# Yukayo/MobGT

Hardware: AMD Instinct MI355X
Metric: check-ins/sec (train step) (higher is better)
Workload: dtype bf16

## Files before the change

__graft_entry__.py:

```python
import os
import subprocess
import sys

ROOT = os.path.dirname(os.path.abspath(__file__))
if ROOT not in sys.path:
    sys.path.insert(0, ROOT)


def build() -> None:
    from mobgt_amd import _native
    for library in _native.LIBRARIES:
        library.build()
        library.lib()
    from mobgt_amd import _pairbins
    _pairbins.LIBRARY.build()
    _pairbins.LIBRARY.lib()
    from mobgt_amd import _universe
    _universe.LIBRARY.build()
    _universe.LIBRARY.lib()
    subprocess.check_call(["make", "-s", "-C", os.path.join(ROOT, "oracle")])
    import mobgt_amd


def smoke() -> None:
    import numpy as np
    import torch
    from mobgt_amd import ops, synth
    from mobgt_amd.model_fqandtoyo import EncoderLayer
    from oracle import algos_oracle as ao
    from oracle import model_oracle as mo
    assert torch.cuda.is_available(), "smoke() needs cuda:0"
    dev = "cuda:0"
    G, H, T, C = 3, 8, 37, 192
    torch.manual_seed(0)
    layer = EncoderLayer(C, 256, 0.1, 0.1, H).eval()
    sd = {"L." + k: v.detach().clone().requires_grad_(True) for k, v in layer.state_dict().items()}
    rng = np.random.RandomState(0)
    x = torch.from_numpy(rng.standard_normal((G, T, C)).astype(np.float32))
    gy = torch.from_numpy(rng.standard_normal((G, T, C)).astype(np.float32))
    bias = torch.from_numpy((rng.standard_normal((G, H, T, T)) * 0.5).astype(np.float32))
    bias[1, :, :, 30:] = float("-inf")
    xr, br = x.clone().requires_grad_(True), bias.clone().requires_grad_(True)
    ref = mo.encoder_layer_fq(sd, "L", xr, br, H)
    ref.backward(gy)
    layer = layer.to(dev)
    xd, bd = x.to(dev).requires_grad_(True), bias.to(dev).requires_grad_(True)
    out = layer(xd, bd)
    out.backward(gy.to(dev))
    torch.cuda.synchronize()

    def close(name, got, want, tol):
        got, want = got.detach().float().cpu().numpy(), want.detach().numpy()
        scale = float(np.sqrt((want ** 2).mean()))
        err = float(np.abs(got - want).max())
        assert err <= tol * scale, f"{name}: max |err| {err:.3e} vs rms {scale:.3e}"
    close("y", out, ref, 1e-3)
    close("dx", xd.grad, xr.grad, 1e-3)
    close("dbias", bd.grad, br.grad, 1e-3)
    for k, p in layer.named_parameters():
        if k.endswith("linear_k.bias"):
            continue
        if sd["L." + k].grad is not None:
            close("d" + k, p.grad, sd["L." + k].grad, 2e-3)
    layer.act_dtype = torch.bfloat16
    for prm in layer.parameters():
        prm.grad = None
    xb, bb = x.to(dev).requires_grad_(True), bias.to(dev).requires_grad_(True)
    out16 = layer(xb, bb)
    out16.backward(gy.to(dev))
    torch.cuda.synchronize()
    close("y (bf16)", out16, ref, 8e-2)
    close("dx (bf16)", xb.grad, xr.grad, 1e-1)
    close("dbias (bf16)", bb.grad, br.grad, 2e-1)
    trajs = synth.make_batch_of_trajectories(seed=4, G=4, P=50, n_user=8, n_nodes=[17, 3, 9, 30])
    n = np.array([len(t["node_name"]) for t in trajs], dtype=np.int32)
    counts = np.zeros((4, 30, 30), dtype=np.int32)
    for g, t in enumerate(trajs):
        counts[g, :n[g], :n[g]] = t["edge_type"]
    sp = ops.spd_batched(torch.from_numpy(counts).to(dev), torch.from_numpy(n).to(dev), 20)
    for g in range(4):
        k = int(n[g])
        M, path = ao.floyd_warshall(counts[g, :k, :k] != 0)
        assert np.array_equal(sp["spd"][g, :k, :k].cpu().numpy().astype(np.int64), M)
        assert np.array_equal(sp["path"][g, :k, :k].cpu().numpy().astype(np.int64), path)
    print("smoke ok: fused fq EncoderLayer fwd+bwd (f32 and bf16 configurations) and batched SPD match the oracle")


if __name__ == "__main__":
    build()
    if len(sys.argv) > 1 and sys.argv[1] == "smoke":
        smoke()
```

mobgt_amd/csrc/tokbwd.hip:

```cpp
#include "common.h"
#include "mobgt_hip.h"

namespace {

typedef __attribute__((ext_vector_type(4))) float f32x4;

constexpr int TNW = 12, TNT = TNW * 64, TBM = 16;

struct TokBwdParams {
    const float* dout;
    const float* real;
    const float* y4;
    const float* y2; int64_t ld2;
    const float *w4, *w2;
    float *d_nf, *d_add;
    float* dx4; int64_t ldx4;
    float* d_pt;
    float* d_token;
    int G, N;
    float slope4, slope2;
    uint32_t thr_pos, thr_in;
    float keep_pos, keep_in;
    uint64_t seed;
    const uint64_t* seed_dev;
    uint32_t salt_nf, salt_tok, salt_in;
    int n_node_blocks;
};

__device__ __forceinline__ float leaky_grad(float y, float slope) { return y > 0.f ? 1.f : slope; }

#ifdef TB_STAMP
__device__ int* g_tb_dbg = nullptr;
#define TSTAMP_DECL int st_[8] = {}
#define TSTAMP(i) st_[i] = (int)wall_clock64()
#define TSTAMP_DUMP() do { if (g_tb_dbg && threadIdx.x == 0) for (int q_ = 0; q_ < 8; ++q_) g_tb_dbg[blockIdx.x * 8 + q_] = st_[q_]; } while (0)
#else
#define TSTAMP_DECL
#define TSTAMP(i)
#define TSTAMP_DUMP()
#endif

template <int N> constexpr int gemm_ks() { return TNW / ((N + 63) / 64); }
template <int K, int N, int LDA, int LDO>
__device__ __forceinline__ void gemm_kn(const float* __restrict__ A, const float* __restrict__ W, float* __restrict__ out) {
    constexpr int NB = (N + 63) / 64, KS = TNW / NB, NT16 = K / 16, TMAX = (NT16 + KS - 1) / KS;
    static_assert(K % 16 == 0 && N % 32 == 0 && KS >= 1, "shape");
    const int lane = threadIdx.x & 63, wave = threadIdx.x >> 6;
    const int j = lane & 15, q = lane >> 4;
    if (wave >= NB * KS) return;
    const int blk = wave / KS, ks = wave % KS;
    const int t_lo = ks * NT16 / KS, t_hi = (ks + 1) * NT16 / KS;
    const int n0 = 64 * blk;
    const bool col_ok = n0 + 4 * j < N;
    const int cl = col_ok ? n0 + 4 * j : 0;
    f32x4 acc[4];
#pragma unroll
    for (int n = 0; n < 4; ++n) acc[n] = f32x4{0.f, 0.f, 0.f, 0.f};
    f32x4 bw[TMAX][4];
#pragma unroll
    for (int tt = 0; tt < TMAX; ++tt) {
        const int t = min(t_lo + tt, t_hi - 1);
#pragma unroll
        for (int i = 0; i < 4; ++i) bw[tt][i] = *reinterpret_cast<const f32x4*>(W + (int64_t)(16 * t + 4 * q + i) * N + cl);
    }
#pragma unroll
    for (int tt = 0; tt < TMAX; ++tt) {
        if (t_lo + tt < t_hi) {
            const f32x4 a = *reinterpret_cast<const f32x4*>(A + j * LDA + 16 * (t_lo + tt) + 4 * q);
#pragma unroll
            for (int i = 0; i < 4; ++i)
#pragma unroll
                for (int n = 0; n < 4; ++n) acc[n] = __builtin_amdgcn_mfma_f32_16x16x4f32(a[i], bw[tt][i][n], acc[n], 0, 0, 0);
        }
    }
    if (col_ok) {
#pragma unroll
        for (int n = 0; n < 4; ++n)
#pragma unroll
            for (int v = 0; v < 4; ++v) out[(ks * TBM + 4 * q + v) * LDO + n0 + 4 * j + n] = acc[n][v];
    }
}

template <int C, int W2>
__global__ __launch_bounds__(TNT) void token_bwd_chain_kernel(const TokBwdParams p) {
    constexpr int LDA = C + 4, LD2 = W2 + 4;
    __shared__ __attribute__((aligned(16))) float a4[TBM * LDA];
    constexpr int KS4 = gemm_ks<C>(), KS2 = gemm_ks<W2>();
    __shared__ __attribute__((aligned(16))) float t4[(KS4 > KS2 ? KS4 : KS2) * TBM * LDA];
    const int lane = threadIdx.x & 63, wave = threadIdx.x >> 6;
    const int T = p.N + 1;
    const uint64_t seed = (p.thr_pos || p.thr_in) ? p.seed + (p.seed_dev ? *p.seed_dev : 0ull) : 0ull;
    if ((int)blockIdx.x >= p.n_node_blocks) {
        const int g = ((int)blockIdx.x - p.n_node_blocks) * TNW + wave;
        if (g >= p.G) return;
        const int64_t row = (int64_t)g * T;
        const uint32_t h1 = p.thr_pos ? dropout_row_hash(seed, (uint32_t)g ^ p.salt_tok) : 0u;
        const uint32_t h2 = p.thr_in ? dropout_row_hash(seed, (uint32_t)row ^ p.salt_in) : 0u;
        for (int c = lane; c < C; c += 64) {
            float scale = 1.f;
            if (p.thr_pos) scale = dropout_bits16(seed, h1, (uint32_t)c) >= p.thr_pos ? p.keep_pos : 0.f;
            if (p.thr_in) scale *= dropout_bits16(seed, h2, (uint32_t)c) >= p.thr_in ? p.keep_in : 0.f;
            const float d = p.dout[row * C + c] * scale;
            if (d != 0.f) atomicAdd(&p.d_token[c], d);
        }
        return;
    }
    const int64_t R = (int64_t)p.G * p.N;
    const int64_t j0 = (int64_t)blockIdx.x * TBM;
    TSTAMP_DECL;
    TSTAMP(0);
    constexpr int EPT = TBM * C / TNT;
    static_assert(TBM * C % TNT == 0, "flat split");
    float dv[EPT], yv[EPT], rl[EPT];
#pragma unroll
    for (int k = 0; k < EPT; ++k) {
        const int e = threadIdx.x + k * TNT, r = e / C, c = e % C;
        const int64_t jc = min(j0 + r, R - 1);
        const int g = (int)(jc / p.N), n = (int)(jc - (int64_t)g * p.N);
        dv[k] = p.dout[((int64_t)g * T + n + 1) * C + c];
        yv[k] = p.y4[jc * C + c];
        rl[k] = p.real[jc];
    }
#pragma unroll
    for (int k = 0; k < EPT; ++k) {
        const int e = threadIdx.x + k * TNT, r = e / C, c = e % C;
        const int64_t jn = j0 + r;
        const bool on = jn < R;
        const int64_t jc = on ? jn : R - 1;
        const int g = (int)(jc / p.N), n = (int)(jc - (int64_t)g * p.N);
        const int64_t row = (int64_t)g * T + n + 1;
        float scale = 1.f;
        if (p.thr_pos) scale = dropout_bits16(seed, dropout_row_hash(seed, (uint32_t)jc ^ p.salt_nf), (uint32_t)c) >= p.thr_pos ? p.keep_pos : 0.f;
        if (p.thr_in) scale *= dropout_bits16(seed, dropout_row_hash(seed, (uint32_t)row ^ p.salt_in), (uint32_t)c) >= p.thr_in ? p.keep_in : 0.f;
        const float d = on ? dv[k] * scale : 0.f;
        const float dnf = d * rl[k];
        a4[r * LDA + c] = dnf * leaky_grad(yv[k], p.slope4);
        if (on) {
            p.d_add[jn * C + c] = d;
            p.d_nf[jn * C + c] = dnf;
        }
    }
    __syncthreads();
    TSTAMP(1);
    gemm_kn<C, C, LDA, LDA>(a4, p.w4, t4);
    __syncthreads();
    TSTAMP(2);
    for (int e = threadIdx.x; e < TBM * C; e += TNT) {
        const int r = e / C, c = e % C;
        const int64_t jn = j0 + r;
        float v = 0.f;
#pragma unroll
        for (int ks = 0; ks < KS4; ++ks) v += t4[(ks * TBM + r) * LDA + c];
        if (jn < R) p.dx4[jn * p.ldx4 + c] = v;
        if (c < W2) a4[r * LD2 + c] = jn < R ? v * leaky_grad(p.y2[jn * p.ld2 + c], p.slope2) : 0.f;
    }
    __syncthreads();
    TSTAMP(3);
    gemm_kn<W2, W2, LD2, LD2>(a4, p.w2, t4);
    __syncthreads();
    TSTAMP(4);
    for (int e = threadIdx.x; e < TBM * W2; e += TNT) {
        const int r = e / W2, c = e % W2;
        const int64_t jn = j0 + r;
        float v = 0.f;
#pragma unroll
        for (int ks = 0; ks < KS2; ++ks) v += t4[(ks * TBM + r) * LD2 + c];
        if (jn < R) p.d_pt[jn * W2 + c] = v;
    }
    TSTAMP(5);
    TSTAMP_DUMP();
}

}

#ifdef TB_STAMP
extern "C" int mobgt_tokbwd_debug_buffer(int* buf) { return (int)hipMemcpyToSymbol(HIP_SYMBOL(g_tb_dbg), &buf, sizeof(buf)); }
#endif

extern "C" int mobgt_token_bwd_chain(const float* dout, const float* real, const float* y4, const float* y2, int64_t ld_y2,
                                     const float* w4, const float* w2, float* d_nf, float* d_add, float* dx4, int64_t ld_dx4,
                                     float* d_pt, float* d_token, int G, int N, int C, int W2, float slope4, float slope2,
                                     float p_pos, float p_in, uint64_t seed, const uint64_t* seed_dev, uint32_t salt_nf,
                                     uint32_t salt_tok, uint32_t salt_in, void* stream) {
    if (G <= 0 || N <= 0) return MOBGT_EBADDIM;
    if (!(C == 192 && W2 == 160)) return MOBGT_EBADDIM;
    if (((uintptr_t)w4 | (uintptr_t)w2) & 15) return MOBGT_EALIGN;
    TokBwdParams p = {};
    p.dout = dout; p.real = real; p.y4 = y4; p.y2 = y2; p.ld2 = ld_y2; p.w4 = w4; p.w2 = w2; p.d_nf = d_nf; p.d_add = d_add;
    p.dx4 = dx4; p.ldx4 = ld_dx4; p.d_pt = d_pt; p.d_token = d_token; p.G = G; p.N = N; p.slope4 = slope4; p.slope2 = slope2;
    p.thr_pos = p_pos > 0.f ? dropout_threshold(p_pos) : 0u;
    p.thr_in = p_in > 0.f ? dropout_threshold(p_in) : 0u;
    p.keep_pos = p.thr_pos ? 1.f / (1.f - (float)p.thr_pos / 65536.f) : 1.f;
    p.keep_in = p.thr_in ? 1.f / (1.f - (float)p.thr_in / 65536.f) : 1.f;
    p.seed = seed; p.seed_dev = seed_dev; p.salt_nf = salt_nf; p.salt_tok = salt_tok; p.salt_in = salt_in;
    p.n_node_blocks = (int)(((int64_t)G * N + TBM - 1) / TBM);
    const dim3 grid(p.n_node_blocks + (G + TNW - 1) / TNW), block(TNT);
    hipLaunchKernelGGL((token_bwd_chain_kernel<192, 160>), grid, block, 0, (hipStream_t)stream, p);
    return (int)hipGetLastError();
}
```

mobgt_amd/forms.py:

```python
import contextlib
import os
from collections import namedtuple

Form = namedtuple("Form", "name env default doc")

_ROWS = (
    Form("safe_forms", "MOBGT_SAFE_FORMS", False, "no launch waits for peer workgroups: one workgroup per row block, the head as "
         "three launches, the GCN layer by layer (what TrainStep.guarded_step switches to before it re-runs a faulted step)"),
    Form("chain", "MOBGT_NO_CHAIN", True, "out-proj -> LN -> FFN -> LN -> the next layer's QKV in one launch (off: separate launches)"),
    Form("chain_big", "MOBGT_NO_CHAIN_BIG", True, "past 4 096 rows: the 64-row forward chain (off: the library's GEMMs)"),
    Form("chain_bwd", None, True, "the same chain backwards, d(out) -> d(attention out)"),
    Form("ln_gemm", None, True, "dropout+residual+LN as the prologue of the GEMM that consumes it (off: the two-launch form)"),
    Form("ln_gemm_bwd", "MOBGT_LN_GEMM_BWD", False, "the LayerNorm-prologue GEMMs in the backward as well"),
    Form("own_gemm", None, True, "the layer's GEMMs on csrc/gemm.hip (off: through torch)"),
    Form("tail", None, True, "a layer's input-gradient GEMM rides in its grouped weight-gradient launch"),
    Form("defer_tail", "MOBGT_NO_DEFER_TAIL", True, "a layer leaves dx and its weight gradients to the chain_bwd launch of the layer "
         "below (off: it finishes its own backward)"),
    Form("wgrad_big", None, True, "past 4 096 rows: the layer's weight gradients as one launch"),
    Form("skinny_all", "MOBGT_SKINNY_ALL", False, "all three classifier products on csrc/skinny.hip (off: dW / db only)"),
    Form("token_fwd_chain", "MOBGT_NO_TOKEN_FWD_CHAIN", True, "the encoder input's forward as one launch (off: four)"),
    Form("token_bwd_chain", "MOBGT_NO_TOKEN_BWD_CHAIN", True, "the encoder input's backward as one launch, csrc/tokbwd.hip (off: three)"),
    Form("pack_passenger", "MOBGT_NO_PACK_PASSENGER", True, "the layers' weight pack, in the next front launch"),
    Form("front_passengers", "MOBGT_NO_FRONT_PASSENGERS", True, "hop table forward and node-feature indices, in the category GCN's forward"),
    Form("bias_bwd_passenger", "MOBGT_NO_BIAS_BWD_PASSENGER", True, "short batches: the bias tables' backward, in the category GCN's backward"),
    Form("bias_bwd_beside", None, True, "long batches: the bias tables' backward on a side stream (off: where autograd reaches it)"),
    Form("l0_ride", "MOBGT_NO_L0_RIDE", True, "the distance GCN's first product, in the bias assembly's launch"),
    Form("psum_defer", "MOBGT_NO_PSUM_DEFER", True, "split-K partial sums, in the step's one reduction launch into the gradient sinks"),
    Form("small_gcn", "MOBGT_NO_SMALL_GCN", True, "the three-layer category GCN as one launch each way (off: layer by layer)"),
    Form("conv_act", "MOBGT_NO_CONV_ACT", True, "bias + LeakyReLU + dropout in the small GEMM's epilogue (off: launch per product)"),
    Form("dist_gcn_fused", "MOBGT_NO_DIST_GCN_FUSED", True, "the distance GCN on the masked-GEMM launches"),
    Form("sp_gather", None, True, "sparse adjacency, transposed product as a gather (off: the atomic scatter)"),
    Form("stock_front", "MOBGT_NO_STOCK_FRONT", True, "hop table, weight pack and encoder input as one front launch"),
    Form("stock_tail", "MOBGT_NO_STOCK_TAIL", True, "the encoder input's and the wide hop table's backward share one grid at the flush"),
    Form("stock_ln_qkv", "MOBGT_NO_STOCK_LN_QKV", True, "the first layer's norm inside its QKV GEMM"),
    Form("attn_one_pass", "MOBGT_ATTN_TWO_PASS", True, "T > 64, bf16: one-pass backward (off: the two deterministic passes)"),
    Form("ddp_overlap", "MOBGT_DDP_OVERLAP", False, "the backward split into graphs, finished gradient slices all-reduced beside the next"),
    Form("ddp_host_exchange", "MOBGT_DDP_HOST_EXCHANGE", False, "all-reduce issued by the host between backward and optimizer graph"),
    Form("force_comm", "MOBGT_FORCE_COMM", False, "a process group of one rank takes the data-parallel path (tests)"),
)
_BY_NAME = {row.name: row for row in _ROWS}
_OVERRIDES = {}


def _env_set(var):
    v = os.environ.get(var, "")
    if v in ("", "0"):
        return False
    if v == "1":
        return True
    raise ValueError(f"{var}={v!r}: expected unset, '', '0' or '1'")


def on(name):
    row = _BY_NAME[name]
    if name in _OVERRIDES:
        return _OVERRIDES[name]
    if row.env is not None and _env_set(row.env):
        return not row.default
    return row.default


def set(name, value):
    _BY_NAME[name]
    if value is None:
        _OVERRIDES.pop(name, None)
    else:
        _OVERRIDES[name] = bool(value)


@contextlib.contextmanager
def using(**names):
    saved = dict(_OVERRIDES)
    try:
        for name, value in names.items():
            set(name, value)
        yield
    finally:
        _OVERRIDES.clear()
        _OVERRIDES.update(saved)


def table():
    return _ROWS
```

mobgt_amd/ops.py:

```python
import contextlib
import ctypes
import math

import torch

from . import _lib, forms
from ._lib import F32, BF16, I64, I32, I16, U8, check
from .step_state import STEP

_DT = {torch.float32: F32, torch.bfloat16: BF16}
_IT = {torch.int64: I64, torch.int32: I32, torch.int16: I16, torch.uint8: U8}


def _stream():
    return ctypes.c_void_p(torch.cuda.current_stream().cuda_stream)


def _p(t):
    return ctypes.c_void_p(t.data_ptr()) if t is not None else ctypes.c_void_p(0)


def _require_cuda(*ts):
    for t in ts:
        if t is not None and not t.is_cuda:
            raise RuntimeError("mobgt_amd ops run on the GPU only (there is no CPU fallback); got a CPU tensor")




def _ws_word(ws, off):
    return ws.view(torch.int32)[off // 4:off // 4 + 1]


def _scrub_exchange_area(ws, fault_off):
    ws[fault_off + 4:].zero_()
    torch.cuda.synchronize()


def peer_wait_faults(reset=True):
    from . import fused_layer
    lib = _lib.lib()
    dev = torch.cuda.current_device()
    torch.cuda.synchronize(dev)
    out = {}
    for key, ws in fused_layer._CHAIN_WS.items():
        if key[0] != dev:
            continue
        off = int(lib.mobgt_chain_ws_fault_offset())
        w = _ws_word(ws, off)
        n = int(w.item())
        if n:
            out["chain"] = out.get("chain", 0) + n
            if reset:
                w.zero_()
                _scrub_exchange_area(ws, off)
    ws = _HEAD_WS.get(dev)
    if ws is not None:
        off = int(lib.mobgt_head_chain_ws_fault_offset())
        w = _ws_word(ws, off)
        n = int(w.item())
        if n:
            out["head"] = n
            if reset:
                w.zero_()
                _scrub_exchange_area(ws, off)
    c = ctypes.c_uint32(0)
    _lib.call("mobgt_small_gcn_faults", 1 if reset else 0, ctypes.byref(c))
    if c.value:
        out["small_gcn"] = int(c.value)
    return out


def set_peer_wait_limit(rounds=0, gcn_ticks=0):
    from . import fused_layer
    lib = _lib.lib()
    dev = torch.cuda.current_device()
    rounds = int(rounds) & 0xFFFFFFFF
    rounds = rounds - (1 << 32) if rounds >= (1 << 31) else rounds
    for key, ws in fused_layer._CHAIN_WS.items():
        if key[0] == dev:
            _ws_word(ws, int(lib.mobgt_chain_ws_limit_offset())).fill_(int(rounds))
    ws = _HEAD_WS.get(dev)
    if ws is not None:
        _ws_word(ws, int(lib.mobgt_head_chain_ws_limit_offset())).fill_(int(rounds))
    _lib.call("mobgt_small_gcn_set_wait_limit", int(gcn_ticks))
    torch.cuda.synchronize()


class ZeroArena:

    def __init__(self, device, n=1 << 20):
        self.buf = torch.zeros(n, dtype=torch.float32, device=device)
        self.off = 0

    def reset(self):
        self.buf.zero_()
        self.off = 0

    def take(self, n):
        n4 = (n + 3) // 4 * 4
        if self.off + n4 > self.buf.numel():
            return None
        t = self.buf[self.off:self.off + n]
        self.off += n4
        return t


def set_zero_arena(arena):
    STEP.zero_arena = arena


def zeros_f32(shape, device):
    n = 1
    for d in (shape if isinstance(shape, (tuple, list, torch.Size)) else (shape,)):
        n *= int(d)
    a = STEP.zero_arena
    if a is not None and a.buf.device == torch.device(device):
        t = a.take(n)
        if t is not None:
            return t.view(shape)
    return torch.zeros(shape, dtype=torch.float32, device=device)


def set_grad_sinks(params, views):
    import weakref
    STEP.grad_sinks = {p.data_ptr(): (weakref.ref(p), v) for p, v in zip(params, views)} if params is not None else {}


def sink_census_begin():
    STEP.sink_census.update(on=True, cur={}, max={})


def sink_census_pass():
    c = STEP.sink_census
    for k, n in c["cur"].items():
        if n > c["max"].get(k, 0):
            c["max"][k] = n
    c["cur"] = {}


def sink_census_end():
    sink_census_pass()
    c = STEP.sink_census
    out, c["on"], c["max"] = c["max"], False, {}
    return out


def grad_sink(param):
    c = STEP.sink_census
    if c["on"]:
        c["cur"][id(param)] = c["cur"].get(id(param), 0) + 1
    e = STEP.grad_sinks.get(param.data_ptr())
    if e is not None and e[0]() is param and e[1].shape == param.shape:
        return e[1]
    return None


def round_up(x, m):
    return (x + m - 1) // m * m


class PackedBias:

    def __init__(self, G, H, T, dtype, device):
        self.G, self.H, self.T = G, H, T
        self.ld = round_up(T, 64)
        self.dtype = dtype
        self.bias = torch.empty(G, H, T, self.ld, dtype=dtype, device=device)
        self.bias_t = torch.empty(G, H, T, self.ld, dtype=dtype, device=device)
        self.dbias = None
        self.n_use = 0
        self.n_bwd = 0
        self.needs_grad = False
        self.token = None
        self.spent = False

    def dense(self):
        return self.bias[..., : self.T].float()

    @property
    def sliced(self):
        return self.dtype == torch.bfloat16

    def grad_buffer(self):
        if self.dbias is None:
            shape = (self.G, self.H, self.T, self.ld)
            if self.sliced:
                self.dbias = torch.empty((max(self.n_use, 1),) + shape, dtype=torch.bfloat16, device=self.bias.device)
            else:
                self.dbias = torch.zeros(shape, dtype=torch.float32, device=self.bias.device)
        return self.dbias

    def next_grad_slice(self):
        buf = self.grad_buffer()
        i = self.n_bwd
        self.n_bwd += 1
        if not self.sliced:
            return buf, 1 if i > 0 else 0
        if i >= buf.shape[0]:
            raise RuntimeError("PackedBias: more attention backward passes than forward uses of this bias")
        return buf[i], 0

    def grad_total(self):
        if self.dbias is None:
            return None
        if self.sliced:
            return self.dbias[: max(self.n_bwd, 1), ..., : self.T].float().sum(0)
        return self.dbias[..., : self.T]


class _PackFn(torch.autograd.Function):
    @staticmethod
    def forward(ctx, src, pack):
        G, H, T = pack.G, pack.H, pack.T
        s = src.expand(G, H, T, T)
        st = s.stride()
        _lib.call("mobgt_bias_pack", _p(s), _DT[s.dtype], st[0], st[1], st[2], st[3], _p(pack.bias), _p(pack.bias_t),
                  _DT[pack.dtype], G, H, T, pack.ld, _stream())
        ctx.pack = pack
        ctx.src_shape = src.shape
        ctx.src_dtype = src.dtype
        ctx.set_materialize_grads(False)
        return zeros_f32((1,), src.device)

    @staticmethod
    def backward(ctx, _g):
        pack = ctx.pack
        pack.spent = True
        if pack.dbias is None:
            return torch.zeros(ctx.src_shape, dtype=ctx.src_dtype, device=pack.bias.device), None
        g = pack.grad_total()
        if tuple(ctx.src_shape) != tuple(g.shape):
            g = g.sum_to_size(ctx.src_shape)
        return g.to(ctx.src_dtype), None


def pack_bias(attn_bias, G, H, T, dtype=None):
    _require_cuda(attn_bias)
    if attn_bias.dtype not in _DT:
        attn_bias = attn_bias.float()
    if attn_bias.dim() == 3:
        attn_bias = attn_bias.unsqueeze(1)
    pack = PackedBias(G, H, T, dtype or attn_bias.dtype, attn_bias.device)
    pack.needs_grad = attn_bias.requires_grad and torch.is_grad_enabled()
    pack.token = _PackFn.apply(attn_bias, pack)
    return pack




def front_deferral(on):
    STEP.front_on = bool(on) and forms.on("front_passengers")


def take_front_jobs():
    hop, ni = STEP.front_hop, STEP.front_ni
    STEP.front_hop = STEP.front_ni = None
    return hop, ni


def flush_front():
    hop, ni = take_front_jobs()
    if hop is not None:
        _lib.call("mobgt_hop_table_fwd", *hop[0], _stream())
    if ni is not None:
        _lib.call("mobgt_node_index", *ni[0], _stream())


def _bias_bwd_alloc(shapes, dev, sinks=(None, None, None, None)):
    return tuple(None if sh is None else (k[:] if (k is not None and tuple(k.shape) == tuple(sh)) else zeros_f32(sh, dev))
                 for sh, k in zip(shapes, sinks))


def take_bias_bwd_job():
    job, STEP.bias_bwd_job = STEP.bias_bwd_job, None
    if job is None or not forms.on("bias_bwd_passenger"):
        return None
    pack = job["pack"]()
    if pack is None or pack.dbias is None or not pack.sliced or pack.n_use < 1 or pack.n_bwd < pack.n_use:
        return None
    G, N, H, D_in, D, F, n_rel, n_poi, n_edge, ld, idx_dt, edge_dt = job["args"]
    if not (idx_dt == I16 and edge_dt == U8 and H == 8 and D > 0 and D <= 20 and F == 1 and G * (N + 1) * (N + 1) < (1 << 20)
            and job["idx"][3] is not None):
        return None
    return job


def bias_bwd_job_args(job):
    pack = job["pack"]()
    outs = _bias_bwd_alloc(job["shapes"], pack.bias.device, job.get("sinks", (None,) * 4))
    attn_bias, rel_pos, poi_pos, edge_input = job["idx"]
    n_sl = max(pack.n_bwd, 1) if pack.sliced else 1
    stride = pack.dbias.stride(0) if pack.sliced else 0
    args = [_p(pack.dbias), _DT[pack.dbias.dtype], n_sl, stride, _p(attn_bias), _p(rel_pos), _p(poi_pos), _p(edge_input),
            _p(outs[0]), _p(outs[1]), _p(outs[2]), _p(outs[3]), *job["args"]]
    return outs, args


class _BuildBiasFn(torch.autograd.Function):
    @staticmethod
    def forward(ctx, rel_table, poi_table, hop_table, vdist, pack, attn_bias, rel_pos, poi_pos, edge_input, D, sinks=(None,) * 4):
        G, N = rel_pos.shape[:2]
        H = rel_table.shape[1]
        has_edge = edge_input is not None and D > 0
        D_in = edge_input.shape[3] if has_edge else 0
        F = edge_input.shape[4] if has_edge else 1
        idx_dt = _IT[rel_pos.dtype]
        edge_dt = _IT[edge_input.dtype] if has_edge else U8
        n_poi = poi_table.shape[0] if poi_table is not None else 0
        n_edge = hop_table.shape[1] if has_edge else 0
        args = (G, N, H, D_in, D if has_edge else 0, F, rel_table.shape[0], n_poi, n_edge, pack.ld, idx_dt, edge_dt)
        _lib.call("mobgt_build_bias", _p(attn_bias), _p(rel_pos), _p(poi_pos), _p(edge_input if has_edge else None), _p(rel_table),
                  _p(poi_table), _p(hop_table if has_edge else None), _p(vdist), _p(pack.bias), _p(pack.bias_t),
                  *args, _DT[pack.dtype], _stream())
        ctx.pack, ctx.args = pack, args
        ctx.set_materialize_grads(False)
        ctx.idx = (attn_bias, rel_pos, poi_pos, edge_input if has_edge else None)
        ctx.shapes = (rel_table.shape, None if poi_table is None else poi_table.shape,
                      hop_table.shape if has_edge else None, vdist.shape)
        import weakref
        ctx.job = dict(pack=weakref.ref(pack), args=args, idx=ctx.idx, shapes=ctx.shapes, done=None, sinks=sinks)
        STEP.bias_bwd_job = ctx.job if pack.needs_grad else None
        return zeros_f32((1,), rel_table.device)

    @staticmethod
    def backward(ctx, _g):
        pack = ctx.pack
        dev = pack.bias.device
        if ctx.job["done"] is not None:
            d_rel, d_poi, d_hop, d_vd = ctx.job["done"]
            ev = ctx.job.pop("done_event", None)
            if ev is not None:
                torch.cuda.current_stream(pack.bias.device).wait_event(ev)
            ctx.job["done"] = None
            return d_rel, d_poi, d_hop, d_vd, None, None, None, None, None, None, None
        if STEP.bias_bwd_job is ctx.job:
            STEP.bias_bwd_job = None
        d_rel, d_poi, d_hop, d_vd = _bias_bwd_alloc(ctx.shapes, dev, ctx.job.get("sinks", (None,) * 4))
        if pack.dbias is not None:
            attn_bias, rel_pos, poi_pos, edge_input = ctx.idx
            a = ctx.args
            n_sl = max(pack.n_bwd, 1) if pack.sliced else 1
            stride = pack.dbias.stride(0) if pack.sliced else 0
            _lib.call("mobgt_build_bias_bwd", _p(pack.dbias), _DT[pack.dbias.dtype], n_sl, stride,
                      _p(attn_bias), _p(rel_pos), _p(poi_pos), _p(edge_input),
                      _p(d_rel), _p(d_poi), _p(d_hop), _p(d_vd), *a, _stream())
        return d_rel, d_poi, d_hop, d_vd, None, None, None, None, None, None, None


def build_bias(attn_bias, rel_pos, poi_pos, edge_input, rel_table, poi_table, hop_table, vdist, D, dtype=torch.float32):
    _require_cuda(attn_bias, rel_pos, rel_table)
    G, N = rel_pos.shape[:2]
    H = rel_table.shape[1]
    pack = PackedBias(G, H, N + 1, dtype, rel_table.device)
    pack.needs_grad = torch.is_grad_enabled() and any(
        t is not None and t.requires_grad for t in (rel_table, poi_table, hop_table, vdist))
    f = lambda t: None if t is None else t.contiguous()
    k_vd = grad_sink(vdist)
    sinks = (grad_sink(rel_table), grad_sink(poi_table) if poi_table is not None else None, None,
             k_vd.view(-1) if (k_vd is not None and k_vd.is_contiguous()) else None)
    pack.token = _BuildBiasFn.apply(f(rel_table.float()), f(None if poi_table is None else poi_table.float()),
                                    f(None if hop_table is None else hop_table.float()), f(vdist.float().reshape(-1)),
                                    pack, f(attn_bias.float()), f(rel_pos), f(poi_pos), f(edge_input), int(D), sinks)
    return pack


_ATTN_ONE_PASS = type("_AttnOnePassView", (), {"__getitem__": lambda self, i: forms.on("attn_one_pass")})()


def _check_rows(*ts):
    for t in ts:
        if t.stride(-1) != 1 or t.stride(-2) % 8 != 0 or t.data_ptr() % 16 != 0:
            raise RuntimeError("mobgt attention: q/k/v rows must be unit-stride, 16-byte aligned, row stride % 8 == 0")


def _lse_alloc(G, H, T, C, dtype, device):
    return torch.empty(lse_numel(G, H, T, C, dtype), dtype=torch.float32, device=device)


def lse_numel(G, H, T, C, dtype):
    n = G * H * T
    extra = (G * T * C + 1) // 2 if dtype == torch.bfloat16 else 0
    return (n + 3) // 4 * 4 + extra


def lse_rows(lse, G, H, T):
    return lse[: G * H * T].view(G, H, T)


def _out_lo_ptr(lse, G, H, T, dtype):
    if dtype != torch.bfloat16:
        return None
    return lse.data_ptr() + 4 * ((G * H * T + 3) // 4 * 4)


def _attn_fwd(q, k, v, pack, scale, p_drop, seed, seed_dev):
    G, T, C = q.shape
    H = pack.H
    out = torch.empty(G, T, C, dtype=q.dtype, device=q.device)
    lse = _lse_alloc(G, H, T, C, q.dtype, q.device)
    _check_rows(q, k, v)
    if pack.needs_grad:
        pack.n_use += 1
    _lib.call("mobgt_attn_bias_fwd", _p(q), _p(k), _p(v), _p(pack.bias), _p(out), _out_lo_ptr(lse, G, H, T, q.dtype), _p(lse), G, H, T, C // H,
              q.stride(1), k.stride(1), v.stride(1), C, pack.ld, scale, p_drop, seed,
              _p(seed_dev), _DT[q.dtype], _DT[pack.dtype], _stream())
    return out, lse


_DQ_ACC = {}
_DQ_ACC_RETIRED = []


def _attn_bwd(q, k, v, out, lse, dout, dq, dk, dv, pack, scale, p_drop, seed, seed_dev):
    G, T, C = q.shape
    H = pack.H
    need = lse_numel(G, H, T, C, q.dtype) if q.dtype == torch.bfloat16 else G * H * T
    if lse.dtype != torch.float32 or lse.numel() < need:
        raise ValueError(f"attention backward: `lse` must be the float32 buffer of {need} elements the "
                         f"forward returned (log-sum-exp rows + the bf16 residual of `out`), got {lse.dtype} x {lse.numel()}")
    dbias = None
    acc = 0
    if pack.needs_grad:
        dbias, acc = pack.next_grad_slice()
    delta = torch.empty(G, H, T, dtype=torch.float32, device=q.device)
    args = (_p(q), _p(k), _p(v), _p(pack.bias), _p(pack.bias_t), _p(out), _out_lo_ptr(lse, G, H, T, q.dtype), _p(lse), _p(dout),
            _p(dq), _p(dk), _p(dv), _p(dbias), _p(delta), G, H, T, C // H,
            q.stride(1), k.stride(1), v.stride(1), C, dq.stride(1), dk.stride(1),
            dv.stride(1), pack.ld, scale, p_drop, seed, _p(seed_dev), acc,
            _DT[dbias.dtype] if dbias is not None else F32, _DT[q.dtype], _DT[pack.dtype])
    if (T > 64 and q.dtype == torch.bfloat16 and pack.dtype == torch.bfloat16 and dbias is not None
            and dbias.dtype == torch.bfloat16 and _ATTN_ONE_PASS[0]):
        key = (str(q.device), int(torch.cuda.current_stream(q.device).cuda_stream), G * T * C)
        ent = _DQ_ACC.get(key)
        if ent is None or ent["busy"]:
            if ent is not None:
                _DQ_ACC_RETIRED.append(ent["buf"])
            ent = _DQ_ACC[key] = dict(buf=torch.zeros(G * T * C, dtype=torch.float32, device=q.device), busy=False)
        ent["busy"] = True
        _lib.call("mobgt_attn_bias_bwd_fused_z", *args, _p(ent["buf"]), _stream())
        ent["busy"] = False
        _bias_bwd_beside(pack)
        return
    _lib.call("mobgt_attn_bias_bwd", *args, _stream())
    _bias_bwd_beside(pack)


_SIDE_STREAMS = {}


def _bias_bwd_beside(pack):
    job = STEP.bias_bwd_job
    if (job is None or not forms.on("bias_bwd_beside") or job["pack"]() is not pack or not pack.sliced or pack.dbias is None
            or pack.n_use < 1 or pack.n_bwd < pack.n_use or job["done"] is not None):
        return
    G, N = job["args"][0], job["args"][1]
    if G * (N + 1) * (N + 1) < (1 << 20) or job["idx"][3] is None:
        return
    dev = pack.bias.device
    main = torch.cuda.current_stream(dev)
    side = _SIDE_STREAMS.get(dev)
    if side is None:
        side = _SIDE_STREAMS[dev] = torch.cuda.Stream(device=dev)
    STEP.bias_bwd_job = None
    outs, args = bias_bwd_job_args(job)
    fork = torch.cuda.Event()
    fork.record(main)
    side.wait_event(fork)
    cus = torch.cuda.get_device_properties(dev).multi_processor_count
    lib = _lib.lib()
    lib.mobgt_build_bias_bwd_set_workgroups(max(1, cus * 3 // 4))
    try:
        _lib.call("mobgt_build_bias_bwd", *args, ctypes.c_void_p(side.cuda_stream))
    finally:
        lib.mobgt_build_bias_bwd_set_workgroups(0)
    done = torch.cuda.Event()
    done.record(side)
    job["done"], job["done_event"] = outs, done


class _AttnFn(torch.autograd.Function):

    @staticmethod
    def forward(ctx, q, k, v, token, pack, scale, p_drop, seed, seed_dev):
        out, lse = _attn_fwd(q, k, v, pack, scale, p_drop, seed, seed_dev)
        ctx.save_for_backward(q, k, v, out, lse)
        ctx.misc = (pack, scale, p_drop, seed, seed_dev)
        return out

    @staticmethod
    def backward(ctx, dout):
        q, k, v, out, lse = ctx.saved_tensors
        pack, scale, p_drop, seed, seed_dev = ctx.misc
        dout = dout.contiguous()
        dq, dk, dv = torch.empty_like(out), torch.empty_like(out), torch.empty_like(out)
        _attn_bwd(q, k, v, out, lse, dout, dq, dk, dv, pack, scale, p_drop, seed, seed_dev)
        return dq, dk, dv, None, None, None, None, None, None


class _AttnQKVFn(torch.autograd.Function):

    @staticmethod
    def forward(ctx, qkv, token, pack, scale, p_drop, seed, seed_dev):
        C = qkv.shape[2] // 3
        q, k, v = qkv[..., :C], qkv[..., C:2 * C], qkv[..., 2 * C:]
        out, lse = _attn_fwd(q, k, v, pack, scale, p_drop, seed, seed_dev)
        ctx.save_for_backward(qkv, out, lse)
        ctx.misc = (pack, scale, p_drop, seed, seed_dev)
        return out

    @staticmethod
    def backward(ctx, dout):
        qkv, out, lse = ctx.saved_tensors
        pack, scale, p_drop, seed, seed_dev = ctx.misc
        C = qkv.shape[2] // 3
        q, k, v = qkv[..., :C], qkv[..., C:2 * C], qkv[..., 2 * C:]
        dqkv = torch.empty_like(qkv)
        _attn_bwd(q, k, v, out, lse, dout.contiguous(), dqkv[..., :C], dqkv[..., C:2 * C], dqkv[..., 2 * C:], pack,
                  scale, p_drop, seed, seed_dev)
        return dqkv, None, None, None, None, None, None


def attention(q, k, v, pack, scale, p_drop=0.0, seed=0, seed_dev=None):
    _require_cuda(q, k, v)
    return _AttnFn.apply(q, k, v, pack.token, pack, float(scale), float(p_drop), int(seed), seed_dev)


def attention_qkv(qkv, pack, scale, p_drop=0.0, seed=0, seed_dev=None):
    _require_cuda(qkv)
    if qkv.shape[2] % 24 != 0:
        raise RuntimeError("fused qkv width must be 3*C with C % 8 == 0")
    return _AttnQKVFn.apply(qkv.contiguous(), pack.token, pack, float(scale), float(p_drop), int(seed), seed_dev)


def dropout_keep_mask(seed, G, H, T, p_drop):
    import numpy as np
    m = np.empty((G, H, T, T), dtype=np.uint8)
    _lib.call("mobgt_attn_dropout_mask_host", int(seed) & 0xFFFFFFFFFFFFFFFF, G, H, T, float(p_drop), m.ctypes.data)
    return m.astype(bool)


def dropout_site_mask(seed, salt, R, C, p_drop, row0=0):
    import numpy as np
    m = np.empty((R, C), dtype=np.uint8)
    _lib.call("mobgt_dropout_mask_host", int(seed) & 0xFFFFFFFFFFFFFFFF, int(salt) & 0xFFFFFFFF, int(row0), R, C, float(p_drop),
              m.ctypes.data)
    return m.astype(bool)


def spd_batched(counts, n_nodes, D):
    _require_cuda(counts, n_nodes)
    G, N = counts.shape[:2]
    dev = counts.device
    out = dict(
        spd=torch.empty(G, N, N, dtype=torch.int16, device=dev), path=torch.empty(G, N, N, dtype=torch.int16, device=dev),
        rel_pos=torch.empty(G, N, N, dtype=torch.int16, device=dev),
        edge_input=torch.empty(G, N, N, D, 1, dtype=torch.uint8, device=dev),
        in_degree=torch.empty(G, N, dtype=torch.int16, device=dev), out_degree=torch.empty(G, N, dtype=torch.int16, device=dev))
    work = torch.empty(int(_lib.lib().mobgt_spd_workspace_bytes(G, N)), dtype=torch.uint8, device=dev)
    _lib.call("mobgt_spd_batched", _p(counts.contiguous()), _p(n_nodes.contiguous()), _p(out["spd"]), _p(out["path"]),
              _p(out["rel_pos"]), _p(out["edge_input"]), _p(out["in_degree"]),
              _p(out["out_degree"]), _p(work), G, N, D, _stream())
    return out


def _ptr_array(ts):
    arr = (ctypes.c_void_p * len(ts))(*[t.data_ptr() for t in ts])
    return arr


class _GatherSumFn(torch.autograd.Function):
    @staticmethod
    def forward(ctx, skip, n_tables, *args):
        tables, idx = args[:n_tables], args[n_tables:]
        R = idx[0].numel()
        C = tables[0].shape[1]
        out = torch.empty(R, C, dtype=torch.float32, device=tables[0].device)
        _lib.call("mobgt_embed_gather_sum", _ptr_array(tables), _ptr_array(idx), n_tables, _p(out), R, C, C,
                  _IT[idx[0].dtype], _stream())
        ctx.idx, ctx.skip = idx, skip
        ctx.shapes = [t.shape for t in tables]
        ptrs = [t.data_ptr() for t in tables]
        ctx.sinks = [grad_sink(t) if ptrs.count(t.data_ptr()) == 1 else None for t in tables]
        return out

    @staticmethod
    def backward(ctx, dout):
        if dout.stride(1) != 1 or dout.stride(0) % 4 or dout.data_ptr() % 16:
            dout = dout.contiguous()
        n = len(ctx.shapes)
        grads = [k[:] if (k is not None and tuple(k.shape) == tuple(s)) else zeros_f32(tuple(s), dout.device)
                 for s, k in zip(ctx.shapes, ctx.sinks)]
        skip = (ctypes.c_int64 * n)(*ctx.skip)
        R, C = dout.shape
        _lib.call("mobgt_embed_scatter_add", _ptr_array(grads), _ptr_array(ctx.idx), skip, n, _p(dout), R, C,
                  dout.stride(0), _IT[ctx.idx[0].dtype], _stream())
        return (None, None, *grads, *([None] * n))


class _HopTableFn(torch.autograd.Function):
    @staticmethod
    def forward(ctx, edge_weight, edge_dis_weight, H, D, fp16_roundtrip):
        E = edge_weight.shape[0]
        ew, dw = edge_weight.contiguous(), edge_dis_weight.contiguous()
        tab = torch.empty(D, E, H, dtype=torch.float32, device=ew.device)
        args = [_p(ew), _p(dw), _p(tab), D, E, H, int(fp16_roundtrip)]
        if STEP.front_on:
            if STEP.front_hop is not None:
                flush_front()
            STEP.front_hop = (args, (ew, dw, tab))
        else:
            _lib.call("mobgt_hop_table_fwd", *args, _stream())
        ctx.save_for_backward(ew, dw)
        ctx.misc = (H, D, int(fp16_roundtrip), edge_dis_weight.shape)
        ctx.sinks = (grad_sink(edge_weight), grad_sink(edge_dis_weight))
        return tab

    @staticmethod
    def backward(ctx, dtab):
        ew, dw = ctx.saved_tensors
        H, D, rt, dis_shape = ctx.misc
        E = ew.shape[0]
        k_e, k_d = ctx.sinks
        d_ew = k_e[:] if k_e is not None else torch.empty_like(ew)
        d_dw = k_d[:] if k_d is not None else zeros_f32(tuple(dis_shape), ew.device)
        dtab = dtab.contiguous()
        park = STEP.wgrad_on and k_e is not None and k_d is not None
        if (park and STEP.wgrad_hop is None and H == 8 and E <= 256 and dtab.data_ptr() % 16 == 0 and dw.data_ptr() % 16 == 0):
            STEP.wgrad_hop = (dtab, ew, dw, d_ew, d_dw, D, E, rt)
            return d_ew[:], d_dw[:], None, None, None
        if (park and STEP.wgrad_hop_wide is None and H == 8 and E <= 2048 and dtab.data_ptr() % 16 == 0 and dw.data_ptr() % 16 == 0
                and forms.on("stock_tail")):
            STEP.wgrad_hop_wide = (dtab, ew, dw, d_ew, d_dw, D, E, rt)
            return d_ew[:], d_dw[:], None, None, None
        _hop_table_bwd((dtab, ew, dw, d_ew, d_dw, D, E, rt), H)
        return d_ew, d_dw, None, None, None


def _hop_table_bwd(job, H=8):
    dtab, ew, dw, d_ew, d_dw, D, E, rt = job
    _lib.call("mobgt_hop_table_bwd", _p(dtab), _p(ew), _p(dw), _p(d_ew), _p(d_dw), D, E, H, rt, _stream())


def hop_table(edge_weight, edge_dis_weight, H, D, fp16_roundtrip=False):
    _require_cuda(edge_weight, edge_dis_weight)
    assert edge_weight.dtype == torch.float32 and edge_dis_weight.dtype == torch.float32
    assert edge_dis_weight.numel() >= D * H * H
    return _HopTableFn.apply(edge_weight, edge_dis_weight, H, D, fp16_roundtrip)


class _SkinnyLinearFn(torch.autograd.Function):
    @staticmethod
    def forward(ctx, x, weight, bias):
        x, w = x.contiguous(), weight.contiguous()
        if x.data_ptr() % 16:
            x = x.clone()
        G, K = x.shape
        V = w.shape[0]
        ctx.all_hip = forms.on("skinny_all")
        if ctx.all_hip:
            y = torch.empty(G, V, dtype=torch.float32, device=x.device)
            _lib.call("mobgt_skinny_linear_fwd", _p(x), _p(w), _p(bias), _p(y), G, K, V, _stream())
        elif K % 64 == 0 and K <= 448:
            y = torch.empty(G, V, dtype=torch.float32, device=x.device)
            _lib.call("mobgt_skinny_linear_fwd_mfma", _p(x), _p(w), _p(bias), _p(y), G, K, V, _stream())
        else:
            y = torch.addmm(bias, x, w.t()) if bias is not None else x @ w.t()
        ctx.save_for_backward(x, w)
        ctx.has_bias = bias is not None
        ctx.sink = grad_sink(weight)
        ctx.sink_b = grad_sink(bias) if bias is not None else None
        return y

    @staticmethod
    def backward(ctx, dy):
        return _skinny_backward(ctx, dy)


def _skinny_backward(ctx, dy):
    x, w = ctx.saved_tensors[:2]
    G, K = x.shape
    V = w.shape[0]
    dy = dy.contiguous()
    dx = None
    dx_mfma = ctx.needs_input_grad[0] and not ctx.all_hip and K % 16 == 0 and K <= 512
    both = dx_mfma and ctx.needs_input_grad[1]
    if dx_mfma:
        dx = zeros_f32((G, K), x.device)
        if not both:
            _lib.call("mobgt_skinny_linear_dx", _p(dy), _p(w), _p(dx), G, K, V, _stream())
    elif ctx.needs_input_grad[0]:
        dx = torch.empty_like(x) if ctx.all_hip else dy @ w
    dw = None
    if ctx.needs_input_grad[1]:
        dw = ctx.sink[:] if ctx.sink is not None else torch.empty_like(w)
    db = None
    if ctx.has_bias and ctx.needs_input_grad[2]:
        db = ctx.sink_b[:] if ctx.sink_b is not None else torch.empty(V, dtype=torch.float32, device=x.device)
    if both:
        _lib.call("mobgt_skinny_linear_bwd_both", _p(dy), _p(x), _p(w), _p(dx), _p(dw), _p(db), G, K, V, _stream())
        return dx, dw, db
    _lib.call("mobgt_skinny_linear_bwd", _p(dy), _p(x), _p(w), _p(dx if ctx.all_hip else None), _p(dw), _p(db),
              G, K, V, _stream())
    return dx, dw, db


class _SkinnyLinearGtlFn(torch.autograd.Function):

    @staticmethod
    def forward(ctx, x, weight, bias, targets, alpha, target_offset, logits_out):
        x, w = x.contiguous(), weight.contiguous()
        if x.data_ptr() % 16:
            x = x.clone()
        G, K = x.shape
        V = w.shape[0]
        dz = torch.empty(G, V, dtype=torch.float32, device=x.device)
        loss = torch.empty((), dtype=torch.float32, device=x.device)
        y = None
        if logits_out is not None:
            y = logits_out.t = torch.empty(G, V, dtype=torch.float32, device=x.device)
        _lib.call("mobgt_skinny_linear_gtl", _p(x), _p(w), _p(bias), _p(targets.long().contiguous()), int(target_offset), _p(y), _p(dz),
                  _p(loss), G, K, V, float(alpha), _stream())
        ctx.save_for_backward(x, w, dz)
        ctx.all_hip = False
        ctx.has_bias = bias is not None
        ctx.sink = grad_sink(weight)
        ctx.sink_b = grad_sink(bias) if bias is not None else None
        return loss

    @staticmethod
    def backward(ctx, g):
        dz = ctx.saved_tensors[2]
        if g.data_ptr() != unit_grad(g.device).data_ptr():
            dz = dz * g
        return (*_skinny_backward(ctx, dz), None, None, None, None)


def skinny_linear_gtl_ok(x, weight):
    return (skinny_linear_ok(x, weight) and x.shape[1] % 64 == 0 and x.shape[1] <= 448)


def skinny_linear_gtl(x, weight, bias, targets, alpha=0.25, target_offset=0, logits_out=None):
    _require_cuda(x, weight, targets)
    return _SkinnyLinearGtlFn.apply(x, weight, bias, targets[: x.shape[0]].reshape(-1), alpha, target_offset, logits_out)


def skinny_linear_ok(x, weight):
    return (x.is_cuda and x.dim() == 2 and x.dtype == torch.float32 and weight.dtype == torch.float32
            and 0 < x.shape[0] <= 16 and x.shape[1] % 4 == 0 and x.shape[1] <= 512 and weight.shape[0] >= 1024
            and weight.is_contiguous() and weight.data_ptr() % 16 == 0)


def skinny_linear(x, weight, bias=None):
    _require_cuda(x, weight)
    return _SkinnyLinearFn.apply(x, weight, bias)


def gather_rows_t(a, rows):
    _require_cuda(a, rows)
    assert a.dtype == torch.bfloat16 and a.stride(1) == 1 and rows.dtype == torch.int64
    R, C = rows.numel(), a.shape[1]
    out = torch.empty(R, C, dtype=a.dtype, device=a.device)
    out_t = torch.empty(C, R, dtype=a.dtype, device=a.device)
    _lib.call("mobgt_gather_rows_t", _p(a), a.stride(0), _p(rows.contiguous()), _p(out), _p(out_t), R, C, _stream())
    return out, out_t


def target_rank(scores, target):
    _require_cuda(scores, target)
    scores = scores.float().contiguous()
    target = target.reshape(-1).long().contiguous()
    G, V = scores.shape
    rank = torch.empty(G, 2, dtype=torch.int32, device=scores.device)
    _lib.call("mobgt_target_rank", _p(scores), _p(target), _p(rank), G, V, _stream())
    return rank


_RANK_WORK, _RANK_WORK_OLD = {}, []


def rank_metrics_work_bytes(G, V):
    return int(_lib.lib().mobgt_rank_metrics_work_bytes(G, V))


def rank_metrics_masked_work_bytes(G, V):
    return int(_lib.lib().mobgt_rank_metrics_masked_work_bytes(G, V))


def _rank_work(device, G, V, work=None, nbytes=None):
    n = rank_metrics_work_bytes(G, V) if nbytes is None else nbytes
    if work is not None:
        assert work.is_cuda and work.numel() * work.element_size() >= n, f"rank metrics: work buffer of {n} bytes needed"
        return work
    key = (device, torch.cuda.current_stream(device).stream_id)
    buf = _RANK_WORK.get(key)
    if buf is None or buf.numel() < n:
        if torch.cuda.is_current_stream_capturing():
            raise RuntimeError("mobgt rank metrics: no work buffer of this size on this stream yet -- pass `work` or run the call "
                               "once eagerly before capturing it")
        if buf is not None:
            _RANK_WORK_OLD.append(buf)
        buf = _RANK_WORK[key] = torch.empty(max(n, 1 << 16), dtype=torch.uint8, device=device)
    return buf


def _check_acc(acc):
    assert acc.is_cuda and acc.dtype == torch.float64 and acc.numel() == 10 and acc.is_contiguous(), \
        "acc: the f64 [10] device accumulator of metrics.new_accumulator"


def rank_metrics(scores, target, acc, target_offset=0, work=None):
    _require_cuda(scores, target, acc)
    _check_acc(acc)
    scores = scores.float().contiguous()
    target = target.reshape(-1).long().contiguous()
    G, V = scores.shape
    assert target.numel() >= G
    work = _rank_work(scores.device, G, V, work)
    _lib.call("mobgt_rank_metrics", _p(scores), _p(target), int(target_offset), G, V, _p(acc), _p(work), _stream())
    return acc


RM_EXCLUDE_HIST, RM_SPLIT = _lib.CONSTANTS["MOBGT_RM_EXCLUDE_HIST"], _lib.CONSTANTS["MOBGT_RM_SPLIT"]


def rank_metrics_masked(scores, target, acc, target_offset=0, allow=None, hist=None, hist_offset=None, exclude_hist=False,
                        split=False, work=None):
    G, V = scores.shape
    hist_offset = -int(target_offset) if hist_offset is None else int(hist_offset)
    if (exclude_hist or split) and hist is None:
        raise ValueError("rank_metrics_masked: exclude_hist / split need the rows' hist ids")
    S = 3 if split else 1
    assert acc.dtype == torch.float64 and acc.shape == (S, 11) and acc.is_contiguous(), \
        f"rank_metrics_masked: acc = metrics.new_restricted_accumulator(device, split={bool(split)}), f64 [{S}, 11]"
    if allow is not None:
        _check_allow(allow, G, V, "rank_metrics_masked")
    if hist is not None:
        assert hist.dim() == 2 and hist.shape[0] == G and hist.dtype in (torch.int32, torch.int64), \
            f"rank_metrics_masked: hist = [{G}, n] int32 / int64 ids"
    target = target.reshape(-1)
    assert target.numel() >= G
    if not (scores.is_cuda and scores.dtype == torch.float32):
        from .metrics import restricted_sums
        acc += restricted_sums(scores, target, target_offset, allow, hist, hist_offset, exclude_hist, split).to(acc.device)
        return acc
    _require_cuda(scores, target, acc)
    scores = scores.contiguous()
    target = target.long().contiguous()
    ld_allow = 0
    if allow is not None:
        allow, ld_allow = _allow_on_device(allow, V, "rank_metrics_masked")
    n_h, ld_h = 0, 0
    if hist is not None:
        assert hist.is_cuda, "rank_metrics_masked: hist on the device"
        if hist.shape[1] and (hist.stride(1) != 1 or hist.stride(0) < hist.shape[1]):
            hist = hist.contiguous()
        n_h, ld_h = hist.shape[1], max(hist.stride(0), hist.shape[1])
    work = _rank_work(scores.device, G, V, work, rank_metrics_masked_work_bytes(G, V))
    flags = (RM_EXCLUDE_HIST if exclude_hist else 0) | (RM_SPLIT if split else 0)
    if ld_allow:
        _lib.call("mobgt_rank_metrics_masked_rows", _p(scores.detach()), _p(target), int(target_offset), G, V, _p(allow), ld_allow,
                  _p(hist), _IT[hist.dtype] if hist is not None else I64, ld_h, n_h,
                  hist_offset, flags, _p(acc), _p(work), _stream())
        return acc
    _lib.call("mobgt_rank_metrics_masked", _p(scores.detach()), _p(target), int(target_offset), G, V, _p(allow), _p(hist),
              _IT[hist.dtype] if hist is not None else I64, ld_h, n_h, hist_offset, flags,
              _p(acc), _p(work), _stream())
    return acc


def skinny_linear_rank_metrics_ok(x, weight):
    return skinny_linear_gtl_ok(x, weight)


def skinny_linear_rank_metrics(x, weight, bias, target, acc, target_offset=0, work=None):
    _require_cuda(x, weight, target, acc)
    _check_acc(acc)
    assert skinny_linear_rank_metrics_ok(x, weight), "skinny_linear_rank_metrics: G <= 16 rows, K % 64 == 0, K <= 448, f32"
    x = x.contiguous()
    if x.data_ptr() % 16:
        x = x.clone()
    G, K = x.shape
    V = weight.shape[0]
    target = target.reshape(-1)[:G].long().contiguous()
    assert target.numel() == G
    b = bias.detach().contiguous() if bias is not None else None
    work = _rank_work(x.device, G, V, work)
    _lib.call("mobgt_skinny_linear_rank_metrics", _p(x.detach()), _p(weight.detach()), _p(b), _p(target), int(target_offset),
              G, K, V, _p(acc), _p(work), _stream())
    return acc


TOPK_MAX = 64
_TOPK_WORK, _TOPK_WORK_OLD = {}, []


def topk_work_bytes(G, V, k):
    return int(_lib.lib().mobgt_topk_work_bytes(G, V, k))


def pack_allow(mask_or_ids, V, offset=0):
    V = int(V)
    m = mask_or_ids
    if m.dtype == torch.bool:
        if m.dim() != 1 or m.numel() != V:
            raise ValueError(f"pack_allow: a bool mask must be [{V}], got {tuple(m.shape)}")
    else:
        if m.dim() != 1 or m.dtype.is_floating_point or m.dtype.is_complex:
            raise ValueError("pack_allow: ids must be a 1-D integer tensor")
        cols = m.long() - int(offset)
        if cols.numel() and bool(((cols < 0) | (cols >= V)).any()):
            raise ValueError(f"pack_allow: ids outside [{offset}, {V + int(offset)}) (offset {offset})")
        m = torch.zeros(V, dtype=torch.bool, device=m.device)
        m[cols] = True
    W = (V + 31) // 32
    bits = torch.zeros(W * 32, dtype=torch.int64, device=m.device)
    bits[:V] = m.long()
    words = (bits.view(W, 32) << torch.arange(32, dtype=torch.int64, device=m.device)).sum(1)
    return torch.where(words >= 1 << 31, words - (1 << 32), words).to(torch.int32)


EARTH_RADIUS_KM = 6371.0
NEAR_LAST, NEAR_ANY = _lib.CONSTANTS["MOBGT_NEAR_LAST"], _lib.CONSTANTS["MOBGT_NEAR_ANY"]
_NEAR_MODES = {"last": NEAR_LAST, "any": NEAR_ANY}


def near_mode(mode):
    if mode not in _NEAR_MODES:
        raise ValueError(f"near: mode must be 'last' or 'any', got {mode!r}")
    return _NEAR_MODES[mode]


def pack_positions(coords_deg, V, offset, radians=False):
    V, offset = int(V), int(offset)
    if coords_deg.dim() != 2 or coords_deg.shape[1] != 2:
        raise ValueError(f"pack_positions: coords_deg must be [P + 1, 2] degrees, got {tuple(coords_deg.shape)}")
    dev = coords_deg.device
    ids = torch.arange(V, device=dev) + offset
    has = (ids >= 1) & (ids < coords_deg.shape[0])
    ll = coords_deg.to(torch.float64)
    ll = (ll if radians else torch.deg2rad(ll))[ids.clamp(0, coords_deg.shape[0] - 1)]
    lat, lon = ll[:, 0], ll[:, 1]
    xyz = torch.stack([torch.cos(lat) * torch.cos(lon), torch.cos(lat) * torch.sin(lon), torch.sin(lat)], 1)
    pos = torch.zeros(V, 4, dtype=torch.float32, device=dev)
    pos[:, :3] = torch.where(has[:, None], xyz, torch.full_like(xyz, float("inf"))).to(torch.float32)
    return pos


def chord2_of_km(r):
    r = float(r)
    if not r >= 0.0:
        raise ValueError(f"chord2_of_km: radius must be >= 0 km, got {r}")
    c = 2.0 * math.sin(min(r, math.pi * EARTH_RADIUS_KM) / (2.0 * EARTH_RADIUS_KM))
    return float(torch.tensor(c * c, dtype=torch.float64).to(torch.float32))


def _near_words_torch(pos, hist, hist_offset, chord2_max, mode, allow):
    V, (G, n) = pos.shape[0], hist.shape
    dev = pos.device
    W = (V + 31) // 32
    near = torch.zeros(G, W * 32, dtype=torch.bool, device=dev)
    h = hist.to(device=dev, dtype=torch.int64)
    col = h - int(hist_offset)
    valid = (h != 0) & (col >= 0) & (col < V)
    if mode == NEAR_LAST and n:
        j = torch.arange(1, n + 1, device=dev)[None, :]
        last = (valid * j).max(1).values - 1
        valid = valid & (j - 1 == last[:, None])
    c2 = torch.tensor(chord2_max, dtype=torch.float32, device=dev)
    p = pos[:, :3].to(torch.float32)
    for g in range(G):
        a = p[col[g][valid[g]]]
        for a0 in range(0, a.shape[0], 64):
            d = p[None, :, :] - a[a0:a0 + 64, None, :]
            d = d * d
            near[g, :V] |= (((d[..., 0] + d[..., 1]) + d[..., 2]) <= c2).any(0)
    bits = near.view(G, W, 32).long() << torch.arange(32, dtype=torch.int64, device=dev)
    words = bits.sum(2)
    words = torch.where(words >= 1 << 31, words - (1 << 32), words).to(torch.int32)
    if allow is not None:
        words &= allow.to(dev)[:W]
    return words


def near_words(pos, hist, hist_offset, chord2_max, mode="last", allow=None, out=None):
    m = near_mode(mode)
    assert pos.dim() == 2 and pos.shape[1] == 4 and pos.dtype == torch.float32, "near_words: pos = pack_positions(...), f32 [V, 4]"
    assert hist.dim() == 2 and hist.dtype in (torch.int32, torch.int64), "near_words: hist = [G, n] int32 / int64 ids"
    V, (G, n) = pos.shape[0], hist.shape
    W = (V + 31) // 32
    if allow is not None:
        assert allow.dtype == torch.int32 and allow.dim() == 1 and allow.numel() >= W, \
            f"near_words: allow = pack_allow(..., {V}) words, int32 [{W}]"
    if out is not None:
        assert out.dtype == torch.int32 and out.dim() == 2 and out.shape[0] == G and out.shape[1] >= W and out.stride(1) == 1 \
            and out.stride(0) >= W and out.device == pos.device, f"near_words: out = int32 [{G}, >= {W}] on pos' device"
    chord2_max = float(chord2_max)
    if not pos.is_cuda:
        words = _near_words_torch(pos, hist, hist_offset, chord2_max, m, allow)
        if out is None:
            return words
        out[:, :W].copy_(words)
        return out
    _require_cuda(pos, hist)
    pos = pos.contiguous()
    if n and (hist.stride(1) != 1 or hist.stride(0) < n):
        hist = hist.contiguous()
    if allow is not None:
        assert allow.is_cuda and allow.is_contiguous(), "near_words: allow words on the device, contiguous"
    if out is None:
        out = torch.empty(G, W, dtype=torch.int32, device=pos.device)
    if G == 0:
        return out
    _lib.call("mobgt_near_words", _p(pos), V, _p(hist), _IT[hist.dtype], max(hist.stride(0), n), n, int(hist_offset), m,
              chord2_max, _p(allow), _p(out), out.stride(0), G, _stream())
    return out


def _check_allow(allow, G, V, who):
    W = (V + 31) // 32
    if allow.dim() == 2:
        assert allow.dtype == torch.int32 and allow.shape[0] == G and allow.shape[1] >= W, \
            f"{who}: per-row allow = near_words(...) words, int32 [{G}, {W}]"
        return
    assert allow.dtype == torch.int32 and allow.dim() == 1 and allow.numel() >= W, \
        f"{who}: allow = pack_allow(..., {V}) words, int32 [{W}]"


def _allow_on_device(allow, V, who):
    if allow.dim() == 2:
        assert allow.is_cuda, f"{who}: allow words on the device"
        if allow.stride(1) != 1 or allow.stride(0) < (V + 31) // 32:
            allow = allow.contiguous()
        return allow, allow.stride(0)
    assert allow.is_cuda and allow.is_contiguous(), f"{who}: allow words on the device, contiguous"
    return allow, 0


def _candidates(G, V, allow, exclude, exclude_offset, device):
    ok = torch.ones(G, V, dtype=torch.bool, device=device)
    if allow is not None:
        cols = torch.arange(V, device=device)
        w = allow.to(device=device, dtype=torch.int64)[..., cols >> 5]
        ok &= ((w >> (cols & 31)) & 1).bool()
    if exclude is not None and exclude.numel():
        e = exclude.to(device=device, dtype=torch.int64)
        c = e - int(exclude_offset)
        hit = (e != 0) & (c >= 0) & (c < V)
        rows = torch.arange(G, device=device)[:, None].expand_as(c)
        ok[rows[hit], c[hit]] = False
    return ok


def topk_rows(scores, k, col_offset=0, work=None, out=None, allow=None, exclude=None, exclude_offset=None):
    G, V = scores.shape
    k = int(k)
    if not 1 <= k <= V:
        raise ValueError(f"topk_rows: k = {k} outside [1, {V}]")
    if allow is not None or exclude is not None:
        return _topk_rows_masked(scores, k, col_offset, work, out, allow, exclude,
                                 col_offset if exclude_offset is None else exclude_offset)
    if not (scores.is_cuda and scores.dtype == torch.float32):
        vals, idx = torch.sort(scores, dim=1, descending=True, stable=True)
        ids, vals = idx[:, :k] + int(col_offset), vals[:, :k]
        if out is None:
            return ids, vals
        out[0].copy_(ids)
        out[1].copy_(vals)
        return out
    if scores.stride(1) != 1 or scores.stride(0) < V:
        scores = scores.contiguous()
    ids, vals = out = _topk_out(scores, G, k, out)
    if G == 0:
        return out
    work = _topk_work(scores, G, V, k, work)
    _lib.call("mobgt_topk_rows", _p(scores.detach()), scores.stride(0), G, V, k, int(col_offset), _p(ids), _p(vals), _p(work),
              _stream())
    return out


def _topk_rows_masked(scores, k, col_offset, work, out, allow, exclude, exclude_offset):
    G, V = scores.shape
    if allow is not None:
        _check_allow(allow, G, V, "topk_rows")
    if exclude is not None:
        assert exclude.dim() == 2 and exclude.shape[0] == G and exclude.dtype in (torch.int32, torch.int64), \
            f"topk_rows: exclude = [{G}, n] int32 / int64 ids"
    if not (scores.is_cuda and scores.dtype == torch.float32):
        sv, si = torch.sort(scores, dim=1, descending=True, stable=True)
        ok = torch.gather(_candidates(G, V, allow, exclude, exclude_offset, scores.device), 1, si)
        order = torch.sort((~ok).to(torch.uint8), dim=1, stable=True)[1][:, :k]
        keep = torch.gather(ok, 1, order)
        ids = torch.where(keep, torch.gather(si, 1, order) + int(col_offset), torch.full_like(order, -1))
        vals = torch.where(keep, torch.gather(sv, 1, order), torch.full_like(order, float("-inf"), dtype=sv.dtype))
        if out is None:
            return ids, vals
        out[0].copy_(ids)
        out[1].copy_(vals)
        return out
    if scores.stride(1) != 1 or scores.stride(0) < V:
        scores = scores.contiguous()
    ld_allow = 0
    if allow is not None:
        allow, ld_allow = _allow_on_device(allow, V, "topk_rows")
    n_ex, ld_ex = 0, 0
    if exclude is not None:
        assert exclude.is_cuda, "topk_rows: exclude on the device"
        if exclude.shape[1] and (exclude.stride(1) != 1 or exclude.stride(0) < exclude.shape[1]):
            exclude = exclude.contiguous()
        n_ex, ld_ex = exclude.shape[1], max(exclude.stride(0), exclude.shape[1])
    ids, vals = out = _topk_out(scores, G, k, out)
    if G == 0:
        return out
    work = _topk_work(scores, G, V, k, work)
    if ld_allow:
        _lib.call("mobgt_topk_rows_masked_rows", _p(scores.detach()), scores.stride(0), G, V, k, int(col_offset), _p(allow),
                  ld_allow, _p(exclude), _IT[exclude.dtype] if exclude is not None else I64,
                  ld_ex, n_ex, int(exclude_offset), _p(ids), _p(vals), _p(work), _stream())
        return out
    _lib.call("mobgt_topk_rows_masked", _p(scores.detach()), scores.stride(0), G, V, k, int(col_offset), _p(allow),
              _p(exclude), _IT[exclude.dtype] if exclude is not None else I64, ld_ex, n_ex,
              int(exclude_offset), _p(ids), _p(vals), _p(work), _stream())
    return out


def _topk_out(scores, G, k, out):
    if out is None:
        out = (torch.empty(G, k, dtype=torch.int64, device=scores.device), torch.empty(G, k, dtype=torch.float32, device=scores.device))
    ids, vals = out
    assert ids.is_cuda and vals.is_cuda and ids.dtype == torch.int64 and vals.dtype == torch.float32 and ids.is_contiguous() \
        and vals.is_contiguous() and ids.shape == (G, k) and vals.shape == (G, k), "topk_rows: out = ([G, k] int64, [G, k] f32)"
    return out


def _topk_work(scores, G, V, k, work):
    n = topk_work_bytes(G, V, k)
    if work is not None:
        assert work.is_cuda and work.numel() * work.element_size() >= n, f"topk_rows: work buffer of {n} bytes needed"
        return work
    key = (scores.device, torch.cuda.current_stream(scores.device).stream_id)
    work = _TOPK_WORK.get(key)
    if work is None or work.numel() < n:
        if torch.cuda.is_current_stream_capturing():
            raise RuntimeError("topk_rows: no work buffer of this size on this stream yet -- pass `work` or run the call "
                               "once eagerly before capturing it")
        if work is not None:
            _TOPK_WORK_OLD.append(work)
        work = _TOPK_WORK[key] = torch.empty(max(n, 1 << 16), dtype=torch.uint8, device=scores.device)
    return work


def node_index(x, time_normal, poi2cat, rows_only, in_degree=None, out_degree=None):
    _require_cuda(x, time_normal, poi2cat)
    assert x.dtype in (torch.int64, torch.int32) and time_normal.dtype == torch.float32 and poi2cat.dtype == torch.int64
    G, N = x.shape
    idx = torch.empty(8, G, N, dtype=torch.int64, device=x.device)
    real = torch.empty(G, N, dtype=torch.float32, device=x.device)
    deg_dt = I64
    if in_degree is not None:
        in_degree, out_degree = in_degree.reshape(G, N).contiguous(), out_degree.reshape(G, N).contiguous()
        assert in_degree.dtype == out_degree.dtype and in_degree.dtype in _IT
        deg_dt = _IT[in_degree.dtype]
    args = [_p(x), _IT[x.dtype], x.stride(0), x.stride(1), _p(time_normal), time_normal.stride(0), time_normal.stride(1), _p(poi2cat),
            _p(in_degree), _p(out_degree), deg_dt, _p(idx), _p(real), G, N, int(bool(rows_only))]
    if STEP.front_on:
        if STEP.front_ni is not None:
            flush_front()
        STEP.front_ni = (args, (x, time_normal, poi2cat, in_degree, out_degree, idx, real))
    else:
        _lib.call("mobgt_node_index", *args, _stream())
    return idx, real


def embed_gather_sum(tables, indices, padding_idx=None):
    _require_cuda(*tables, *indices)
    n = len(tables)
    shape = indices[0].shape
    skip = tuple(-1 if (padding_idx is None or padding_idx[t] is None) else int(padding_idx[t]) for t in range(n))
    idx = [i.contiguous().reshape(-1) for i in indices]
    tabs = [t.float().contiguous() for t in tables]
    out = _GatherSumFn.apply(skip, n, *tabs, *idx)
    return out.view(*shape, tabs[0].shape[1])


class _GatherConcatFn(torch.autograd.Function):
    @staticmethod
    def forward(ctx, skip, n_tables, *args):
        tables, idx = args[:n_tables], args[n_tables:]
        R = idx[0].numel()
        widths = [t.shape[1] for t in tables]
        ctot = sum(widths)
        out = torch.empty(R, ctot, dtype=torch.float32, device=tables[0].device)
        warr = (ctypes.c_int * n_tables)(*widths)
        _lib.call("mobgt_embed_gather_concat", _ptr_array(tables), _ptr_array(idx), warr, n_tables, _p(out), R, ctot,
                  _IT[idx[0].dtype], _stream())
        ctx.idx, ctx.skip, ctx.widths = idx, skip, widths
        ctx.shapes = [t.shape for t in tables]
        return out

    @staticmethod
    def backward(ctx, dout):
        dout = dout.contiguous()
        n = len(ctx.shapes)
        R, ctot = dout.shape
        grads = [zeros_f32(tuple(s), dout.device) for s in ctx.shapes]
        skip = (ctypes.c_int64 * n)(*ctx.skip)
        warr = (ctypes.c_int * n)(*ctx.widths)
        _lib.call("mobgt_embed_scatter_concat", _ptr_array(grads), _ptr_array(ctx.idx), skip, warr, n, _p(dout), R, ctot,
                  _IT[ctx.idx[0].dtype], _stream())
        return (None, None, *grads, *([None] * n))


def embed_gather_concat(tables, indices, padding_idx=None):
    _require_cuda(*tables, *indices)
    n = len(tables)
    shape = indices[0].shape
    skip = tuple(-1 if (padding_idx is None or padding_idx[t] is None) else int(padding_idx[t]) for t in range(n))
    idx = [i.contiguous().reshape(-1) for i in indices]
    tabs = [t.float().contiguous() for t in tables]
    out = _GatherConcatFn.apply(skip, n, *tabs, *idx)
    return out.view(*shape, out.shape[1])


_ROW0_PENDING = {}


def token_fwd_deferral(on):
    flush_token_fwd()
    STEP.token_fwd_on = bool(on) and forms.on("token_fwd_chain") and not _NAN_TRACE["on"]


def flush_token_fwd():
    for k in ("gather", "f2", "f4"):
        rec = STEP.token_fwd.pop(k, None)
        if rec is not None:
            rec["launch"]()


class _GatherMultiFn(torch.autograd.Function):

    @staticmethod
    def forward(ctx, spec, out_widths, n, *args):
        tables, idx = args[:n], args[n:]
        R = idx[0].numel()
        dev = tables[0].device
        outs = [torch.empty(R, w, dtype=torch.float32, device=dev) for w in out_widths]
        ci, i64, vp = ctypes.c_int, ctypes.c_int64, ctypes.c_void_p

        def launch():
            _lib.call("mobgt_embed_gather_multi",
                n, _ptr_array(tables), None, _ptr_array(idx), (i64 * n)(*[sp[3] for sp in spec]),
                (ci * n)(*[t.shape[1] for t in tables]), (ci * n)(*[sp[1] for sp in spec]), (ci * n)(*[int(sp[2]) for sp in spec]),
                (vp * n)(*[outs[sp[0]].data_ptr() for sp in spec]), (i64 * n)(*[outs[sp[0]].stride(0) for sp in spec]), R,
                _IT[idx[0].dtype], 0, None, 0, _stream())
        if STEP.token_fwd_on and "gather" not in STEP.token_fwd and len(outs) == 3 and all(i_.dtype == idx[0].dtype for i_ in idx):
            STEP.token_fwd["gather"] = dict(launch=launch, tables=tables, idx=idx, spec=spec, outs=outs, R=R)
        else:
            launch()
        ctx.idx, ctx.spec, ctx.n = idx, spec, n
        ctx.ptrs = [t.data_ptr() for t in tables]
        ctx.shapes = [t.shape for t in tables]
        ctx.sinks = [grad_sink(t) for t in tables]
        return tuple(outs)

    @staticmethod
    def backward(ctx, *douts):
        n, spec = ctx.n, ctx.spec
        dev = ctx.idx[0].device
        R = ctx.idx[0].numel()
        gbuf = []
        for g in douts:
            if g is not None and (g.stride(1) != 1 or g.stride(0) % 4 or g.data_ptr() % 16 or g.dtype != torch.float32):
                g = g.float().contiguous()
            gbuf.append(g)
        grads = [(ctx.sinks[t][:] if ctx.sinks[t] is not None else zeros_f32(tuple(sh), dev))
                 if (ctx.needs_input_grad[3 + t] and gbuf[spec[t][0]] is not None) else None for t, sh in enumerate(ctx.shapes)]
        jobs = [t for t in range(n) if grads[t] is not None]
        if jobs:
            m = len(jobs)
            ci, i64, vp = ctypes.c_int, ctypes.c_int64, ctypes.c_void_p
            extra, extra_job = None, 0
            for k, t in enumerate(jobs):
                pend = _ROW0_PENDING.pop(ctx.ptrs[t], None)
                if pend is not None:
                    extra, extra_job = pend, k
            _lib.call("mobgt_embed_gather_multi",
                m, None, (vp * m)(*[grads[t].data_ptr() for t in jobs]), (vp * m)(*[ctx.idx[t].data_ptr() for t in jobs]),
                (i64 * m)(*[spec[t][3] for t in jobs]), (ci * m)(*[ctx.shapes[t][1] for t in jobs]),
                (ci * m)(*[spec[t][1] for t in jobs]), None, (vp * m)(*[gbuf[spec[t][0]].data_ptr() for t in jobs]),
                (i64 * m)(*[gbuf[spec[t][0]].stride(0) for t in jobs]), R, _IT[ctx.idx[0].dtype], 1, _p(extra), extra_job,
                _stream())
        return (None, None, None, *grads, *([None] * n))


def embed_gather_multi(jobs, out_widths):
    n = len(jobs)
    tabs = [j[0].float().contiguous() for j in jobs]
    idx = [j[1].contiguous().reshape(-1) for j in jobs]
    _require_cuda(*tabs, *idx)
    spec = tuple((int(j[2]), int(j[3]), int(j[4]), -1 if j[5] is None else int(j[5])) for j in jobs)
    for k, sp in enumerate(spec):
        assert sp[2] != 2 or (k > 0 and tabs[k].shape[1] == tabs[k - 1].shape[1] and not tabs[k].requires_grad
                              and (k < 4 or any(s_[2] != 2 for s_ in spec[k - 3:k]))), "fold job (at most three per gather)"
    return list(_GatherMultiFn.apply(spec, tuple(out_widths), n, *tabs, *idx))


class _JoinColsFn(torch.autograd.Function):

    @staticmethod
    def forward(ctx, whole, part):
        ctx.w = part.shape[1]
        return whole.detach().view_as(whole)

    @staticmethod
    def backward(ctx, g):
        return g, g[:, :ctx.w]


def join_cols(whole, part):
    return _JoinColsFn.apply(whole, part)


class _GradientTailLossFn(torch.autograd.Function):
    @staticmethod
    def forward(ctx, logits, targets, alpha, target_offset):
        logits = logits.float().contiguous()
        G, V = logits.shape
        dlogits = torch.empty_like(logits)
        loss = torch.empty((), dtype=torch.float32, device=logits.device)
        _lib.call("mobgt_gradient_tail_loss", _p(logits), _p(targets.long().contiguous()), int(target_offset), _p(dlogits),
                  _p(loss), G, V, float(alpha), _stream())
        ctx.save_for_backward(dlogits)
        return loss

    @staticmethod
    def backward(ctx, g):
        (dlogits,) = ctx.saved_tensors
        if g.data_ptr() == unit_grad(g.device).data_ptr():
            return dlogits, None, None, None
        return dlogits * g, None, None, None


class _StockTokensFn(torch.autograd.Function):
    @staticmethod
    def forward(ctx, x, din, dout, atom, indeg, outdeg, gtok, p, seed, seed_dev, salt, padding_idx):
        G, N = x.shape
        C = atom.shape[1]
        y = torch.empty(G, N + 1, C, dtype=torch.float32, device=atom.device)
        tok = (_p(x), _p(din), _p(dout), _IT[x.dtype], _IT[din.dtype], _p(atom), _p(indeg), _p(outdeg), _p(gtok), _p(y),
               G, N, C, atom.shape[0], indeg.shape[0], outdeg.shape[0], p, seed, _p(seed_dev), salt)
        hop, ni = take_front_jobs() if STEP.front_on else (None, None)
        if ni is not None:
            _lib.call("mobgt_node_index", *ni[0], _stream())
        jobs = []
        if STEP.front_on:
            from .model import take_pending_pack
            jobs = take_pending_pack()
        if hop is not None or jobs:
            import ctypes
            vp, ci = ctypes.c_void_p, ctypes.c_int
            for o in range(96, len(jobs), 96):
                from .model import _launch_pack
                _launch_pack(jobs[o:o + 96])
            part = jobs[:96]
            nj = len(part)
            pack = ((vp * nj)(*[j[0].data_ptr() for j in part]), (vp * nj)(*[j[1].data_ptr() for j in part]), (ci * nj)(*[j[2] for j in part]),
                    (ci * nj)(*[j[3] for j in part]), (ci * nj)(*[j[4] for j in part])) if nj else (None, None, None, None, None)
            hargs = [1] + hop[0] if hop is not None else [0, None, None, None, 0, 0, 0, 0]
            _lib.call("mobgt_stock_front_fwd", *tok, nj, *pack, *hargs, _stream())
        else:
            _lib.call("mobgt_stock_tokens_fwd", *tok, _stream())
        ctx.idx = (x, din, dout)
        ctx.misc = (p, seed, seed_dev, salt, padding_idx, [t.shape for t in (atom, indeg, outdeg, gtok)])
        ptrs = [t.data_ptr() for t in (atom, indeg, outdeg, gtok)]
        ctx.sinks = [grad_sink(t) if ptrs.count(t.data_ptr()) == 1 else None for t in (atom, indeg, outdeg, gtok)]
        return y

    @staticmethod
    def backward(ctx, dy):
        x, din, dout = ctx.idx
        p, seed, seed_dev, salt, padding_idx, shapes = ctx.misc
        G, N = x.shape
        dy = dy.contiguous()
        C = dy.shape[2]
        grads = [None if not need else (k[:] if (k is not None and tuple(k.shape) == tuple(sh)) else zeros_f32(tuple(sh), dy.device))
                 for need, k, sh in zip(ctx.needs_input_grad[3:7], ctx.sinks, shapes)]
        args = [_p(dy), _p(x), _p(din), _p(dout), _IT[x.dtype], _IT[din.dtype], _p(grads[0]), _p(grads[1]), _p(grads[2]),
                _p(grads[3]), G, N, C, shapes[0][0], shapes[1][0], shapes[2][0], int(padding_idx), p, seed, _p(seed_dev), salt]
        in_sinks = all((not need) or (k is not None and tuple(k.shape) == tuple(sh))
                       for need, k, sh in zip(ctx.needs_input_grad[3:7], ctx.sinks, shapes))
        if STEP.wgrad_on and in_sinks and STEP.wgrad_stock_tok is None and forms.on("stock_tail"):
            STEP.wgrad_stock_tok = (args, (dy, x, din, dout, seed_dev, grads))
            return (None, None, None, *[g_[:] if g_ is not None else None for g_ in grads], None, None, None, None, None)
        _lib.call("mobgt_stock_tokens_bwd", *args, _stream())
        return (None, None, None, *grads, None, None, None, None, None)


def stock_tokens_ok(x, atom, indeg, outdeg, gtok):
    return (x.is_cuda and x.dim() == 2 and x.dtype in _IT and atom.shape[1] % 4 == 0
            and all(t.dtype == torch.float32 and t.is_contiguous() and t.data_ptr() % 16 == 0 for t in (atom, indeg, outdeg, gtok)))


def stock_tokens(x, in_degree, out_degree, atom, indeg, outdeg, graph_token, p, training, salt, padding_idx=0):
    _require_cuda(x, atom)
    assert in_degree.dtype == out_degree.dtype and in_degree.dtype in _IT and in_degree.dtype != torch.uint8 and x.dtype != torch.uint8
    if not training:
        p = 0.0
    seed, seed_dev = _DROPOUT_STATE["seed"], _DROPOUT_STATE["seed_dev"]
    if seed_dev is None and p > 0:
        seed = (seed + int(torch.randint(0, 2 ** 31 - 1, (1,)).item())) & 0x7FFFFFFFFFFFFFFF
    return _StockTokensFn.apply(x.contiguous(), in_degree.contiguous(), out_degree.contiguous(), atom, indeg, outdeg, graph_token,
                                float(p), int(seed), seed_dev, int(salt) & 0xFFFFFFFF, int(padding_idx))


class _TokenLayerNormFn(torch.autograd.Function):
    @staticmethod
    def forward(ctx, enc, weight, bias, eps):
        enc = enc.contiguous()
        G, T, C = enc.shape
        y = torch.empty(G, C, dtype=torch.float32, device=enc.device)
        stat = torch.empty(2, G, dtype=torch.float32, device=enc.device)
        _lib.call("mobgt_token_ln_fwd", _p(enc), _p(weight), _p(bias), _p(y), _p(stat[0]), _p(stat[1]), G, T, C, float(eps),
                  _stream())
        ctx.save_for_backward(enc, weight, stat)
        ctx.sinks = (grad_sink(weight), grad_sink(bias))
        return y

    @staticmethod
    def backward(ctx, dy):
        enc, weight, stat = ctx.saved_tensors
        G, T, C = enc.shape
        denc = torch.empty_like(enc)
        dg, db = (k[:] if k is not None else zeros_f32((C,), enc.device) for k in ctx.sinks)
        _lib.call("mobgt_token_ln_bwd", _p(dy.contiguous()), _p(enc), _p(stat[0]), _p(stat[1]), _p(weight), _p(denc), _p(dg), _p(db),
                  G, T, C, _stream())
        return denc, dg, db, None


def token_layer_norm_ok(enc, weight):
    return (enc.is_cuda and enc.dim() == 3 and enc.dtype == torch.float32 and weight.dtype == torch.float32
            and enc.shape[2] <= 1024)


def token_layer_norm(enc, weight, bias, eps=1e-5):
    _require_cuda(enc, weight, bias)
    return _TokenLayerNormFn.apply(enc, weight.contiguous(), bias.contiguous(), eps)


class _CrossEntropyFn(torch.autograd.Function):
    @staticmethod
    def forward(ctx, logits, targets, ignore_index):
        logits = logits.float().contiguous()
        G, V = logits.shape
        dlogits = torch.empty_like(logits)
        loss = torch.empty((), dtype=torch.float32, device=logits.device)
        _lib.call("mobgt_cross_entropy", _p(logits), _p(targets.long().contiguous()), int(ignore_index), _p(dlogits), _p(loss), G, V,
                  _stream())
        ctx.save_for_backward(dlogits)
        return loss

    @staticmethod
    def backward(ctx, g):
        (dlogits,) = ctx.saved_tensors
        if g.data_ptr() == unit_grad(g.device).data_ptr():
            return dlogits, None, None
        return dlogits * g, None, None


def cross_entropy_ok(logits, targets):
    return (logits.is_cuda and logits.dim() == 2 and 0 < logits.shape[0] <= 4095 and logits.shape[1] <= 10240
            and targets.numel() == logits.shape[0])


def cross_entropy(logits, targets, ignore_index=-100):
    _require_cuda(logits, targets)
    return _CrossEntropyFn.apply(logits, targets.reshape(-1), ignore_index)


_UNIT = {}


def unit_grad(device):
    device = torch.device(device)
    key = (device.type, device.index if device.index is not None else (torch.cuda.current_device() if device.type == "cuda" else 0))
    t = _UNIT.get(key)
    if t is None:
        t = torch.ones((), dtype=torch.float32, device=device)
        _UNIT[key] = t
    return t


def gradient_tail_loss(logits, targets, alpha=0.25, target_offset=0):
    _require_cuda(logits, targets)
    return _GradientTailLossFn.apply(logits, targets[: logits.shape[0]].reshape(-1), alpha, target_offset)


class OutRef:

    def __init__(self, t):
        self.t = t.detach()


def register_token_chain(nf, x4, w2_width, w4, slope4, w2, slope2):
    STEP.token_chain = None
    if not forms.on("token_bwd_chain"):
        return
    if (nf.is_cuda and nf.dtype == torch.float32 and x4.dtype == torch.float32 and nf.dim() == 2 and nf.is_contiguous()
            and x4.is_contiguous() and tuple(nf.shape) == tuple(x4.shape) and nf.shape[1] == 192 and w2_width == 160
            and tuple(w4.shape) == (192, 192) and tuple(w2.shape) == (160, 160) and w4.is_contiguous() and w2.is_contiguous()
            and w4.dtype == torch.float32 and w2.dtype == torch.float32):
        STEP.token_chain = dict(nf_ptr=nf.data_ptr(), nf=nf.detach(), x4=x4.detach(), w4=w4.detach(), slope4=float(slope4),
                                w2=w2.detach(), slope2=float(slope2))


def _token_park_linear(g, w, y):
    pend = STEP.token_pending.get(g.data_ptr())
    if pend is None:
        return None
    ent = pend["ent"]
    if pend["stage"] == 1 and w.data_ptr() == ent["w4"].data_ptr() and y is not None and y.data_ptr() == ent["nf_ptr"]:
        del STEP.token_pending[g.data_ptr()]
        dx4 = torch.empty_like(ent["x4"])
        pend.update(stage=2, dx4=dx4)
        STEP.token_pending[dx4.data_ptr()] = pend
        return dx4
    if pend["stage"] == 2 and w.data_ptr() == ent["w2"].data_ptr() and y is not None and y.data_ptr() == ent["x4"].data_ptr():
        del STEP.token_pending[g.data_ptr()]
        G, N, C, p_pos, p_in, seed, seed_dev, salts = pend["misc"]
        W2 = ent["w2"].shape[0]
        d_pt = torch.empty(G * N, W2, dtype=torch.float32, device=g.device)
        dx4 = pend["dx4"]
        _lib.call("mobgt_token_bwd_chain", _p(pend["dout"]), _p(pend["real"]), _p(ent["nf"]), _p(ent["x4"]), ent["x4"].stride(0),
                  _p(ent["w4"]), _p(ent["w2"]), _p(pend["d_nf"]), _p(pend["d_add"]), _p(dx4), dx4.stride(0),
                  _p(d_pt), _p(pend["d_tok"]), G, N, C, W2, ent["slope4"], ent["slope2"], p_pos, p_in, seed,
                  _p(seed_dev), salts[0], salts[1], salts[2], _stream())
        return d_pt
    return None


class _LinearSplitKFn(torch.autograd.Function):

    @staticmethod
    def forward(ctx, x, w, b, bf16_wgrad, slope, out=None):
        ctx.bf16_wgrad = bf16_wgrad
        ctx.slope = slope
        if _small_linear(x, w) & 1:
            rec, gat = STEP.token_fwd, STEP.token_fwd.get("gather") if STEP.token_fwd_on else None
            stage = None
            if gat is not None and slope is not None and b is not None and x.dtype == torch.float32 and w.dtype == torch.float32:
                if ("f2" not in rec and out is not None and x.data_ptr() == gat["outs"][0].data_ptr()
                        and out.t.data_ptr() == gat["outs"][1].data_ptr()):
                    stage = "f2"
                elif ("f2" in rec and "f4" not in rec and out is None
                        and x.data_ptr() == gat["outs"][1].data_ptr() and x.is_contiguous()):
                    stage = "f4"
            if stage is not None:
                y = out.t if out is not None else torch.empty(x.shape[0], w.shape[0], dtype=torch.float32, device=x.device)
                rec[stage] = dict(launch=lambda: small_gemm(x, w, b, True, leaky=slope, out=y), x=x, w=w, b=b, slope=slope, y=y)
            else:
                y = small_gemm(x, w, b, True, leaky=slope, out=out.t if out is not None else None)
            if out is not None:
                y = y.view_as(y)
        else:
            y = torch.addmm(b, x, w.t())
            if slope is not None:
                y = torch.nn.functional.leaky_relu(y, slope)
        ctx.save_for_backward(x, w, y if slope is not None else None)
        ctx.sinks = (grad_sink(w), grad_sink(b) if b is not None else None)
        return y

    @staticmethod
    def backward(ctx, g):
        x, w, y = ctx.saved_tensors
        k_w, k_b = ctx.sinks

        def dst(sink, shape):
            return sink[:] if sink is not None else zeros_f32(shape, g.device)
        if y is None or y.is_contiguous():
            g = g.contiguous()
        R = x.shape[0]
        hip_wgrad = (ctx.bf16_wgrad and g.dtype == torch.float32 and x.dtype == torch.float32 and g.shape[1] % 2 == 0
                     and x.shape[1] % 2 == 0 and R <= 4096 and g.data_ptr() % 8 == 0 and x.data_ptr() % 8 == 0)
        if y is not None:
            mv = act_mask_values(ctx.slope, 0.0)
            if (hip_wgrad and R <= 64 and small_gemm_ok(g, w) and y.is_contiguous() and y.data_ptr() % 8 == 0
                    and max(w.shape) <= 512):
                db = dst(k_b, (g.shape[1],))
                dw = linear_wgrad_masked(g, x, g_mask=y, mask_vals=mv, db=db, leaf=True, dw=dst(k_w, tuple(w.shape)))
                dx = _token_park_linear(g, w, y) if STEP.wgrad_on else None
                return (dx if dx is not None else small_gemm(g, w, a_mask=(y, *mv))), dw, (db[:] if STEP.wgrad_on else db), None, None, None
            if (STEP.wgrad_on and hip_wgrad and g.stride(1) == 1 and y.stride() == g.stride() and g.data_ptr() % 8 == 0
                    and y.data_ptr() % 8 == 0 and g.stride(0) % 2 == 0 and small_gemm_ok(g, w) and R <= _SMALL_ROWS
                    and max(w.shape) <= 512):
                db = dst(k_b, (g.shape[1],))
                dw = linear_wgrad_masked(g, x, g_mask=y, mask_vals=mv, db=db, leaf=True, dw=dst(k_w, tuple(w.shape)))
                dx = _token_park_linear(g, w, y)
                return (dx if dx is not None else small_gemm(g, w, a_mask=(y, *mv))), dw, db[:], None, None, None
            if (hip_wgrad and g.stride(1) == 1 and y.stride() == g.stride() and g.data_ptr() % 8 == 0 and y.data_ptr() % 8 == 0
                    and g.stride(0) % 2 == 0):
                gm = torch.empty_strided(g.shape, g.stride(), dtype=torch.float32, device=g.device)
                db = zeros_f32((g.shape[1],), g.device)
                dw = linear_wgrad_masked(g, x, g_mask=y, mask_vals=mv, db=db, g_out=gm)
                dx = small_gemm(gm, w) if (small_gemm_ok(gm, w) and R <= _SMALL_ROWS and max(w.shape) <= 512) else gm @ w
                return dx, dw, db, None, None, None
            g = torch.ops.aten.leaky_relu_backward(g, y, ctx.slope, True).contiguous()
        if hip_wgrad:
            dw, db = linear_wgrad(g, x, with_bias=True, leaf=True, dw=dst(k_w, tuple(w.shape)), db=dst(k_b, (g.shape[1],)))
            return (small_gemm(g, w) if _small_linear(g, w) & 2 else g @ w), dw, db, None, None, None
        s = max((c for c in (16, 8, 4, 2) if R % c == 0 and R // c >= 16), default=1)
        if s > 1:
            dw = torch.bmm(g.view(s, R // s, -1).transpose(1, 2), x.view(s, R // s, -1)).sum(0)
        else:
            dw = g.t() @ x
        return g @ w, dw, colsum(g), None, None, None


_SMALL_LINEAR = 1
_SMALL_ROWS = 4096


def _small_linear(x, w):
    ok = (x.is_cuda and x.dtype == torch.float32 and w.dtype == torch.float32 and x.dim() == 2 and x.shape[0] <= _SMALL_ROWS
          and max(w.shape) <= 512 and x.stride(1) == 1 and w.is_contiguous())
    if not ok:
        return 0
    return _SMALL_LINEAR if x.shape[0] <= 64 else (_SMALL_LINEAR & 1)


def linear_splitk(x, weight, bias, bf16_wgrad=False, slope=None, out=None):
    shape = x.shape
    x2 = x.reshape(-1, shape[-1]).contiguous()
    if out is not None and not (_small_linear(x2, weight) & 1 and out.shape == (x2.shape[0], weight.shape[0])):
        out = None
    y = _LinearSplitKFn.apply(x2, weight, bias, bf16_wgrad, slope, OutRef(out) if out is not None else None)
    return y if out is not None else y.view(*shape[:-1], weight.shape[0])


_DROPOUT_STATE = {"seed_dev": None, "seed": 0x5DEECE66D}


def set_dropout_state(seed_dev=None, seed=None):
    _DROPOUT_STATE["seed_dev"] = seed_dev
    if seed is not None:
        _DROPOUT_STATE["seed"] = int(seed)


class _DropoutFn(torch.autograd.Function):
    @staticmethod
    def forward(ctx, x, p, seed, seed_dev, salt):
        x = x.contiguous()
        y = torch.empty_like(x)
        row = x.shape[-1] if x.dim() > 1 else x.numel()
        _lib.call("mobgt_dropout", _p(x), _p(y), x.numel(), row, p, seed, _p(seed_dev), salt, _stream())
        ctx.misc = (p, seed, seed_dev, salt, row)
        return y

    @staticmethod
    def backward(ctx, g):
        p, seed, seed_dev, salt, row = ctx.misc
        g = g.contiguous()
        dx = torch.empty_like(g)
        _lib.call("mobgt_dropout", _p(g), _p(dx), g.numel(), row, p, seed, _p(seed_dev), salt, _stream())
        return dx, None, None, None, None


def dropout(x, p, training, salt):
    if not training or p <= 0.0:
        return x
    _require_cuda(x)
    seed, seed_dev = _DROPOUT_STATE["seed"], _DROPOUT_STATE["seed_dev"]
    if seed_dev is None:
        seed = (seed + int(torch.randint(0, 2 ** 31 - 1, (1,)).item())) & 0x7FFFFFFFFFFFFFFF
    return _DropoutFn.apply(x.float(), float(p), int(seed), seed_dev, int(salt) & 0xFFFFFFFF)


class _BiasActFn(torch.autograd.Function):
    @staticmethod
    def forward(ctx, x, bias, slope, p_drop, seed, seed_dev, salt, yt=None):
        x = x.contiguous()
        R, C = x.shape
        y = torch.empty_like(x)
        _lib.call("mobgt_bias_act_fwd_t", _p(x), _p(bias), _p(y), _p(yt.t if yt is not None else None),
                  yt.t.stride(0) if yt is not None else 0, R, C, slope, p_drop, seed, _p(seed_dev), salt,
                  _stream())
        ctx.save_for_backward(y)
        ctx.misc = (slope, p_drop, seed, seed_dev, salt, bias is not None)
        return y

    @staticmethod
    def backward(ctx, dy):
        (y,) = ctx.saved_tensors
        slope, p_drop, seed, seed_dev, salt, has_bias = ctx.misc
        R, C = y.shape
        dx = torch.empty_like(y)
        db = zeros_f32((C,), y.device) if has_bias else None
        _lib.call("mobgt_bias_act_bwd", _p(dy.contiguous()), _p(y), _p(dx), _p(db), R, C, slope, p_drop, seed, _p(seed_dev),
                  salt, _stream())
        return dx, db, None, None, None, None, None, None


def dropout_seed(p_drop):
    seed, seed_dev = _DROPOUT_STATE["seed"], _DROPOUT_STATE["seed_dev"]
    if seed_dev is None and p_drop > 0:
        seed = (seed + int(torch.randint(0, 2 ** 31 - 1, (1,)).item())) & 0x7FFFFFFFFFFFFFFF
    return int(seed), seed_dev


def bias_act(x, bias, slope, p_drop, training, salt, yt=None):
    _require_cuda(x)
    if not training:
        p_drop = 0.0
    seed, seed_dev = _DROPOUT_STATE["seed"], _DROPOUT_STATE["seed_dev"]
    if seed_dev is None and p_drop > 0:
        seed = (seed + int(torch.randint(0, 2 ** 31 - 1, (1,)).item())) & 0x7FFFFFFFFFFFFFFF
    return _BiasActFn.apply(x.float(), bias, float(slope), float(p_drop), int(seed), seed_dev, int(salt) & 0xFFFFFFFF,
                            OutRef(yt) if yt is not None else None)


class _HeadActFn(torch.autograd.Function):
    @staticmethod
    def forward(ctx, u, w, b, eps, slope, p_drop, seed, seed_dev, salt):
        u, w, b = u.contiguous(), w.contiguous(), b.contiguous()
        R, C = u.shape
        out = torch.empty_like(u)
        stats = torch.empty(2, R, dtype=torch.float32, device=u.device)
        _lib.call("mobgt_head_act_fwd", _p(u), _p(w), _p(b), _p(out), _p(stats[0]), _p(stats[1]), R, C, eps, slope, p_drop,
                  seed, _p(seed_dev), salt, _stream())
        ctx.save_for_backward(u, w, b, stats)
        ctx.misc = (eps, slope, p_drop, seed, seed_dev, salt)
        return out

    @staticmethod
    def backward(ctx, dout):
        u, w, b, stats = ctx.saved_tensors
        eps, slope, p_drop, seed, seed_dev, salt = ctx.misc
        R, C = u.shape
        du = torch.empty_like(u)
        dg, db = zeros_f32((C,), u.device), zeros_f32((C,), u.device)
        _lib.call("mobgt_head_act_bwd", _p(dout.contiguous()), _p(u), _p(w), _p(b), _p(stats[0]), _p(stats[1]), _p(du),
                  _p(dg), _p(db), R, C, eps, slope, p_drop, seed, _p(seed_dev), salt, _stream())
        return du, dg, db, None, None, None, None, None, None


def head_act(u, ln_weight, ln_bias, eps, slope, p_drop, training, salt):
    _require_cuda(u, ln_weight, ln_bias)
    if not training:
        p_drop = 0.0
    seed, seed_dev = _DROPOUT_STATE["seed"], _DROPOUT_STATE["seed_dev"]
    if seed_dev is None and p_drop > 0:
        seed = (seed + int(torch.randint(0, 2 ** 31 - 1, (1,)).item())) & 0x7FFFFFFFFFFFFFFF
    return _HeadActFn.apply(u.float(), ln_weight, ln_bias, float(eps), float(slope), float(p_drop), int(seed), seed_dev,
                            int(salt) & 0xFFFFFFFF)


class _HeadChainFn(torch.autograd.Function):

    @staticmethod
    def forward(ctx, enc, table, user, offset, w3, b3, ln_w, ln_b, eps, slope, p_drop, seed, seed_dev, salt, bf16_wgrad):
        G, T, C = enc.shape
        U = table.shape[1]
        W = C + U
        dev = enc.device
        x3, u3, out = (torch.empty(G, W, dtype=torch.float32, device=dev) for _ in range(3))
        stats = torch.empty(2, G, dtype=torch.float32, device=dev)
        _lib.call("mobgt_head_chain_fwd", _p(enc), _p(user), _IT[user.dtype], offset, _p(table), table.shape[0], _p(w3), _p(b3),
                  _p(ln_w), _p(ln_b), _p(x3), _p(u3), _p(out), _p(stats[0]), _p(stats[1]), G, T, C, U,
                  eps, slope, p_drop, seed, _p(seed_dev), salt, _p(_head_chain_ws(dev)), _stream())
        ctx.save_for_backward(x3, u3, stats, w3, ln_w, ln_b)
        ctx.user = user
        ctx.misc = (G, T, C, U, offset, tuple(table.shape), eps, slope, p_drop, seed, seed_dev, salt, bf16_wgrad)
        ctx.sink = grad_sink(table)
        ctx.psinks = (grad_sink(w3), grad_sink(b3), grad_sink(ln_w), grad_sink(ln_b))
        return out

    @staticmethod
    def backward(ctx, dout):
        x3, u3, stats, w3, ln_w, ln_b = ctx.saved_tensors
        G, T, C, U, offset, tshape, eps, slope, p_drop, seed, seed_dev, salt, bf16_wgrad = ctx.misc
        dev = dout.device
        dout = dout.contiguous()
        du3 = torch.empty_like(u3)
        denc = torch.empty(G, T, C, dtype=torch.float32, device=dev)
        dtable = ctx.sink[:] if ctx.sink is not None else zeros_f32(tshape, dev)
        k_w3, k_b3, k_g, k_beta = ctx.psinks
        dg = k_g[:] if k_g is not None else zeros_f32((C + U,), dev)
        dbeta = k_beta[:] if k_beta is not None else zeros_f32((C + U,), dev)
        _lib.call("mobgt_head_chain_bwd", _p(dout), _p(u3), _p(stats[0]), _p(stats[1]), _p(ctx.user), _IT[ctx.user.dtype], offset,
                  tshape[0], _p(w3), _p(ln_w), _p(ln_b), _p(du3), _p(denc), _p(dtable), _p(dg), _p(dbeta),
                  G, T, C, U, eps, slope, p_drop, seed, _p(seed_dev), salt, _stream())
        if bf16_wgrad:
            dw, db = linear_wgrad(du3, x3, with_bias=True, leaf=True, dw=k_w3[:] if k_w3 is not None else None,
                                  db=k_b3[:] if k_b3 is not None else None)
        else:
            dw, db = du3.t() @ x3, colsum(du3)
        return denc, dtable, None, None, dw, db, dg, dbeta, None, None, None, None, None, None, None


_HEAD_WS = {}


def _head_chain_ws(dev):
    key = dev.index if dev.index is not None else torch.cuda.current_device()
    ws = _HEAD_WS.get(key)
    if ws is None:
        if torch.cuda.is_current_stream_capturing():
            raise RuntimeError("the head kernel's workspace must be allocated before graph capture: run one eager step first")
        ws = _HEAD_WS[key] = torch.zeros(int(_lib.lib().mobgt_head_chain_ws_bytes()), dtype=torch.uint8, device=dev)
    return ws


def head_chain_ok(enc, table, user, w3):
    W = enc.shape[-1] + table.shape[1]
    return (enc.is_cuda and enc.dim() == 3 and enc.dtype == torch.float32 and table.dtype == torch.float32 and table.is_contiguous()
            and W in (320, 384) and tuple(w3.shape) == (W, W) and w3.dtype == torch.float32 and w3.is_contiguous()
            and user.dtype in (torch.int64, torch.int32) and user.numel() == enc.shape[0] and enc.shape[0] <= 160
            and enc.shape[-1] % 16 == 0 and table.shape[1] % 16 == 0 and not forms.on("safe_forms"))


def head_chain(enc, user_table, user, user_offset, w3, b3, ln_weight, ln_bias, eps, slope, p_drop, training, salt, bf16_wgrad=False):
    _require_cuda(enc, user_table, user, w3)
    if not training:
        p_drop = 0.0
    seed, seed_dev = _DROPOUT_STATE["seed"], _DROPOUT_STATE["seed_dev"]
    if seed_dev is None and p_drop > 0:
        seed = (seed + int(torch.randint(0, 2 ** 31 - 1, (1,)).item())) & 0x7FFFFFFFFFFFFFFF
    return _HeadChainFn.apply(enc.contiguous(), user_table, user.reshape(-1).contiguous(), int(user_offset), w3, b3.contiguous(),
                              ln_weight.contiguous(), ln_bias.contiguous(), float(eps), float(slope), float(p_drop), int(seed),
                              seed_dev, int(salt) & 0xFFFFFFFF, bool(bf16_wgrad))


class _HeadInputFn(torch.autograd.Function):
    @staticmethod
    def forward(ctx, enc, table, user, offset):
        G, T, C = enc.shape
        U = table.shape[1]
        x3 = torch.empty(G, C + U, dtype=torch.float32, device=enc.device)
        _lib.call("mobgt_head_input_fwd", _p(enc), _p(user), _IT[user.dtype], offset, _p(table), table.shape[0], _p(x3),
                  G, T, C, U, _stream())
        ctx.user, ctx.misc = user, (G, T, C, U, offset, table.shape)
        ctx.sink = grad_sink(table)
        return x3

    @staticmethod
    def backward(ctx, dx3):
        G, T, C, U, offset, tshape = ctx.misc
        dx3 = dx3.contiguous()
        denc = torch.empty(G, T, C, dtype=torch.float32, device=dx3.device)
        dtable = ctx.sink[:] if ctx.sink is not None else zeros_f32(tuple(tshape), dx3.device)
        _lib.call("mobgt_head_input_bwd", _p(dx3), _p(ctx.user), _IT[ctx.user.dtype], offset, _p(denc), _p(dtable),
                  tshape[0], G, T, C, U, _stream())
        return denc, dtable, None, None


def head_input(enc, user_table, user, user_offset=0):
    _require_cuda(enc, user_table, user)
    assert enc.dtype == torch.float32 and user_table.dtype == torch.float32 and user.dtype in (torch.int64, torch.int32)
    assert user_table.is_contiguous()
    return _HeadInputFn.apply(enc.contiguous(), user_table, user.reshape(-1).contiguous(), int(user_offset))


def _token_fwd_fused(nf, real, add, token, pe0, out, out16, qkv_w, qkv, G, N, C, p_pos, p_in, seed, seed_dev, salts):
    gat, f2, f4 = (STEP.token_fwd.get(k) for k in ("gather", "f2", "f4"))
    ok = (gat is not None and f2 is not None and f4 is not None and C == 192 and gat["R"] == G * N and len(gat["outs"]) == 3
          and nf.data_ptr() == f4["y"].data_ptr() and add.data_ptr() == gat["outs"][2].data_ptr()
          and tuple(f2["w"].shape) == (160, 160) and tuple(f4["w"].shape) == (192, 192)
          and gat["outs"][0].shape[1] == 160 and gat["outs"][1].shape[1] == 192 and gat["outs"][2].shape[1] == 192
          and all(t.is_contiguous() for t in (f2["w"], f2["b"], f4["w"], f4["b"], *gat["outs"]))
          and (pe0.dim() == 1 or pe0.shape[0] >= 1))
    if not ok:
        flush_token_fwd()
        return False
    tables, idx, spec = gat["tables"], gat["idx"], gat["spec"]
    n = len(tables)
    ci = ctypes.c_int
    rc = (_lib.lib().mobgt_token_fwd_chain(
        n, _ptr_array(tables), _ptr_array(idx), (ci * n)(*[t.shape[1] for t in tables]), (ci * n)(*[sp[1] for sp in spec]),
        (ci * n)(*[int(sp[2]) for sp in spec]), (ci * n)(*[sp[0] for sp in spec]), _IT[idx[0].dtype],
        _p(gat["outs"][0]), _p(gat["outs"][1]), _p(gat["outs"][2]), _p(f4["y"]), 160,
        _p(f2["w"]), _p(f2["b"]), float(f2["slope"]), _p(f4["w"]), _p(f4["b"]), float(f4["slope"]),
        _p(real), _p(token), _p(pe0), _p(out), _p(out16), _p(qkv_w[0].t), _p(qkv_w[1].t), _p(qkv), G, N, C, p_pos, p_in, seed,
        _p(seed_dev), salts[0], salts[1], salts[2], _stream()))
    if rc == _lib.CONSTANTS["MOBGT_EBADDIM"]:
        flush_token_fwd()
        return False
    check(rc, "mobgt_token_fwd_chain")
    STEP.token_fwd = {}
    STEP.token_fwd_fused_calls += 1
    return True


class _AssembleTokensFn(torch.autograd.Function):
    @staticmethod
    def forward(ctx, nf, real, add, token, pe0, p_pos, p_in, seed, seed_dev, salts, side, row0_via_gather=False, qkv_w=None, tok_sink=None):
        ctx.tok_sink = tok_sink
        ctx.pe_ptr = pe0.data_ptr() if (row0_via_gather and pe0.dim() == 2 and pe0.shape[0] > 1) else None
        ctx.nf_ptr = nf.data_ptr()
        G, N, C = nf.shape
        nf, add, real = nf.contiguous(), add.contiguous(), real.contiguous()
        shapes = (token.shape, pe0.shape)
        token = token.reshape(-1).contiguous()
        pe0 = pe0.contiguous() if pe0.dim() == 2 and pe0.shape[0] > 1 else pe0.reshape(-1).contiguous()
        out = torch.empty(G, N + 1, C, dtype=torch.float32, device=nf.device)
        out16 = torch.empty(G, N + 1, C, dtype=torch.bfloat16, device=nf.device) if side is not None else None
        if qkv_w is not None and out16 is not None and C in (192, 256):
            qkv = torch.empty(G * (N + 1), 3 * C, dtype=torch.bfloat16, device=nf.device)
            if not _token_fwd_fused(nf, real, add, token, pe0, out, out16, qkv_w, qkv, G, N, C, p_pos, p_in, seed, seed_dev, salts):
                _lib.call("mobgt_assemble_tokens_qkv", _p(nf), _p(real), _p(add), _p(token), _p(pe0), _p(out), _p(out16),
                          _p(qkv_w[0].t), _p(qkv_w[1].t), _p(qkv), G, N, C, p_pos, p_in, seed,
                          _p(seed_dev), salts[0], salts[1], salts[2], _stream())
            side.append(out16)
            side.append(qkv)
        else:
            flush_token_fwd()
            _lib.call("mobgt_assemble_tokens_fwd", _p(nf), _p(real), _p(add), _p(token), _p(pe0), _p(out), _p(out16), G, N, C,
                      p_pos, p_in, seed, _p(seed_dev), salts[0], salts[1], salts[2], _stream())
            if side is not None:
                side.append(out16)
        ctx.save_for_backward(real)
        ctx.misc = (G, N, C, p_pos, p_in, seed, seed_dev, salts, shapes)
        return out

    @staticmethod
    def backward(ctx, dout):
        (real,) = ctx.saved_tensors
        G, N, C, p_pos, p_in, seed, seed_dev, salts, (tshape, pshape) = ctx.misc
        dout = dout.contiguous()
        d_nf = torch.empty(G, N, C, dtype=torch.float32, device=dout.device)
        d_add = torch.empty(G, N, C, dtype=torch.float32, device=dout.device)
        k_tok = ctx.tok_sink
        if ctx.pe_ptr is not None:
            d_tok = k_tok.view(-1)[:] if (k_tok is not None and k_tok.numel() == C) else zeros_f32((C,), dout.device)
            d_pe = None
        elif len(pshape) == 2 and pshape[0] > 1:
            d_pe = zeros_f32(tuple(pshape), dout.device)
            d_tok = d_pe[0]
        else:
            d_tok = zeros_f32((C,), dout.device)
            d_pe = d_tok.view(pshape)
        ent = STEP.token_chain
        if (ent is not None and ent["nf_ptr"] == ctx.nf_ptr and STEP.wgrad_on and C == ent["nf"].shape[1]
                and G * N == ent["nf"].shape[0] and forms.on("token_bwd_chain")):
            STEP.token_pending[d_nf.data_ptr()] = dict(stage=1, ent=ent, dout=dout, real=real, d_nf=d_nf, d_add=d_add, d_tok=d_tok,
                                                       misc=(G, N, C, p_pos, p_in, seed, seed_dev, salts))
        else:
            _lib.call("mobgt_assemble_tokens_bwd", _p(dout), _p(real), _p(d_nf), _p(d_add), _p(d_tok), G, N, C, p_pos, p_in, seed,
                      _p(seed_dev), salts[0], salts[1], salts[2], _stream())
        if ctx.pe_ptr is not None:
            _ROW0_PENDING[ctx.pe_ptr] = d_tok
            return d_nf, None, d_add, d_tok.view(tshape), None, None, None, None, None, None, None, None, None, None
        return d_nf, None, d_add, d_tok.view(tshape), d_pe, None, None, None, None, None, None, None, None, None


def assemble_tokens(nf, real, add, token, pe0, p_pos, p_in, training, salts=(0x1001, 0x1002, 0x1003), bf16_copy=False,
                    pe_row0_via_gather=False, first_qkv=None):
    _require_cuda(nf, add, token, pe0)
    if not training:
        p_pos = p_in = 0.0
    seed, seed_dev = _DROPOUT_STATE["seed"], _DROPOUT_STATE["seed_dev"]
    if seed_dev is None and (p_pos > 0 or p_in > 0):
        seed = (seed + int(torch.randint(0, 2 ** 31 - 1, (1,)).item())) & 0x7FFFFFFFFFFFFFFF
    side = [] if bf16_copy else None
    out = _AssembleTokensFn.apply(nf.float(), real.float(), add.float(), token.float(), pe0.float(), float(p_pos),
                                  float(p_in), int(seed), seed_dev, tuple(int(s) & 0xFFFFFFFF for s in salts), side,
                                  bool(pe_row0_via_gather and pe0.requires_grad and torch.is_grad_enabled()),
                                  (OutRef(first_qkv[0]), OutRef(first_qkv[1])) if (first_qkv is not None and bf16_copy) else None,
                                  grad_sink(token) if token.is_contiguous() else None)
    if side:
        out._mobgt_act = side[0]
        if len(side) > 1:
            out._mobgt_qkv = side[1]
    return out


def small_gemm(a, b, bias=None, b_is_nk=False, out=None, out_dtype=torch.float32, leaky=None, drop=None, a_mask=None, ct=None,
               k_b=None):
    _require_cuda(a, b)
    assert a.dtype == torch.float32 and b.dtype == torch.float32 and a.dim() == 2 and b.dim() == 2
    assert a.stride(1) == 1 and b.stride(1) == 1
    pre = STEP.front_sgemm.get("done")
    if pre is not None:
        if (pre["key"] == (a.data_ptr(), b.data_ptr(), bias.data_ptr() if bias is not None else 0, leaky, k_b,
                           ct[0].data_ptr() if ct else 0) and drop is None and a_mask is None and out is None and not b_is_nk):
            del STEP.front_sgemm["done"]
            return pre["c"]
    M, K = a.shape
    N = b.shape[0] if b_is_nk else b.shape[1]
    assert (b.shape[1] if b_is_nk else b.shape[0]) == (K if k_b is None else k_b) and (k_b is None or (not b_is_nk and k_b <= K))
    if bias is not None:
        assert bias.dtype == torch.float32 and bias.numel() == N and bias.is_contiguous()
    only_t = ct is not None and ct[2]
    c = None if only_t else (out if out is not None else torch.empty(M, N, dtype=out_dtype, device=a.device))
    if leaky is None and a_mask is None and ct is None and k_b is None:
        _lib.call("mobgt_small_gemm_f32", _p(a), a.stride(0), _p(b), b.stride(0), int(b_is_nk), _p(bias), _p(c), c.stride(0),
                  _DT[c.dtype], M, N, K, _stream())
        return c
    y, pos, neg, zer = a_mask if a_mask is not None else (None, 1.0, 1.0, 1.0)
    if y is not None:
        assert y.dtype == torch.float32 and y.shape == a.shape and y.stride(1) == 1 and y.stride(0) == a.stride(0)
    p_drop, seed, seed_dev, salt = drop if drop is not None else (0.0, 0, None, 0)
    _lib.call("mobgt_small_gemm_f32_act", _p(a), a.stride(0), _p(y), float(pos), float(neg), float(zer), _p(b), b.stride(0),
              int(b_is_nk), _p(bias), int(leaky is not None), float(leaky or 0.0), float(p_drop),
              int(seed), _p(seed_dev), int(salt) & 0xFFFFFFFF, _p(c), c.stride(0) if c is not None else N,
              _DT[c.dtype] if c is not None else F32, _p(ct[0] if ct else None),
              ct[0].stride(0) if ct else 0, _p(ct[1] if ct else None), M, N, K, int(k_b or 0),
              _stream())
    return c


def front_small_gemm(a, b, bias, leaky, k_b, ct):
    STEP.front_sgemm = {}
    if (not forms.on("l0_ride") or not (a.is_cuda and a.dtype == torch.float32 and b.dtype == torch.float32
            and a.is_contiguous() and b.is_contiguous() and bias is not None and bias.is_contiguous())):
        return False
    M, K = a.shape
    N = b.shape[1]
    c = torch.empty(M, N, dtype=torch.float32, device=a.device)
    rc = _lib.lib().mobgt_front_sgemm_job(_p(a), a.stride(0), _p(b), b.stride(0), _p(bias), 1, float(leaky), _p(c), c.stride(0),
                                          _p(ct), ct.stride(0) if ct is not None else 0, M, N, K, int(k_b))
    if rc != 0:
        return False
    STEP.front_sgemm["job"] = dict(key=(a.data_ptr(), b.data_ptr(), bias.data_ptr(), leaky, k_b, ct.data_ptr() if ct is not None else 0),
                                   c=c, args=(a, b, bias, leaky, k_b, ct))
    return True


def front_small_gemm_flush():
    job = STEP.front_sgemm.pop("job", None)
    if job is None:
        return
    if _lib.lib().mobgt_front_sgemm_pending():
        _lib.call("mobgt_front_sgemm_job", None, 0, None, 0, None, 0, 0.0, None, 0, None, 0, 0, 0, 0, 0)
        a, b, bias, leaky, k_b, ct = job["args"]
        job["c"] = small_gemm(a, b, bias, leaky=leaky, k_b=k_b, ct=(ct, None, False) if ct is not None else None)
    STEP.front_sgemm["done"] = job


def graph_task_id():
    fn = getattr(torch._C, "_current_graph_task_id", None)
    return int(fn()) if fn is not None else -1


def drop_parked():
    if "job" in STEP.front_sgemm:
        _lib.call("mobgt_front_sgemm_job", None, 0, None, 0, None, 0, 0.0, None, 0, None, 0, 0, 0, 0, 0)
    STEP.drop_parked(graph_task_id())


def act_mask_values(slope, p_drop):
    if p_drop and p_drop > 0.0:
        thr = int(p_drop * 65536.0 + 0.5)
        ik = 1.0 / (1.0 - thr / 65536.0)
        return ik, slope * ik, 0.0
    return 1.0, slope, slope


@contextlib.contextmanager
def recording_wgrads(on=True):
    STEP.wgrad_on = bool(on)
    try:
        yield
        flush_deferred_wgrads()
    except BaseException:
        drop_parked()
        raise
    finally:
        STEP.wgrad_on = False


def defer_partial_sum(part, dst):
    if not (STEP.wgrad_on and dst is not None and part.dtype == torch.float32 and dst.dtype == torch.float32
            and part.is_contiguous() and dst.is_contiguous() and part.dim() == 3 and dst.numel() == part[0].numel()
            and dst.numel() % 4 == 0 and part.data_ptr() % 16 == 0 and dst.data_ptr() % 16 == 0
            and forms.on("psum_defer")):
        return None
    STEP.wgrad_psum.append((part, dst))
    return dst[:]


def layer_wgrad_big(items, R):
    lib = _lib.lib()
    n = len(items)
    vp, i64, ci = ctypes.c_void_p, ctypes.c_int64, ctypes.c_int
    tiles = sum(lib.mobgt_layer_wgrad_big_tiles(g.shape[1], x.shape[1]) for g, x, _, _ in items)
    S = lib.mobgt_layer_wgrad_big_splits(R, tiles)
    dev = items[0][0].device
    parts = [torch.empty(S, g.shape[1], x.shape[1], dtype=torch.float32, device=dev) for g, x, _, _ in items]
    _lib.call("mobgt_layer_wgrad_big", n, (vp * n)(*[t[0].data_ptr() for t in items]), (i64 * n)(*[t[0].stride(0) for t in items]),
              (vp * n)(*[t[1].data_ptr() for t in items]), (i64 * n)(*[t[1].stride(0) for t in items]),
              (vp * n)(*[q.data_ptr() for q in parts]),
              (vp * n)(*[(t[2].data_ptr() if t[2] is not None else None) for t in items]),
              (ci * n)(*[t[0].shape[1] for t in items]), (ci * n)(*[t[1].shape[1] for t in items]), R, S,
              _stream())
    outs = []
    for part, (_, _, _, sink) in zip(parts, items):
        parked = defer_partial_sum(part, sink) if sink is not None else None
        outs.append(parked if parked is not None else part.sum(0))
    return outs


def layer_wgrad_big_ok(items):
    return (1 <= len(items) <= 4 and all(
        g.dtype == torch.bfloat16 and x.dtype == torch.bfloat16 and g.dim() == 2 and x.dim() == 2 and g.shape[0] == x.shape[0]
        and g.stride(1) == 1 and x.stride(1) == 1 and g.shape[1] % 8 == 0 and x.shape[1] % 8 == 0 and g.stride(0) % 8 == 0
        and x.stride(0) % 8 == 0 and g.data_ptr() % 16 == 0 and x.data_ptr() % 16 == 0
        and g.shape[0] * g.stride(0) * 2 < (1 << 31) and x.shape[0] * x.stride(0) * 2 < (1 << 31) for g, x, _, _ in items))


def _wgrad_defer(g, x, g_mask, x_mask, mask_vals, dw, db, db_of_x):
    STEP.wgrad_items.append((g, x, g_mask, x_mask, tuple(float(v) for v in mask_vals), dw, db, bool(db_of_x)))
    return dw[:]


def step_state_leftovers():
    return STEP.leftovers()


def flush_deferred_wgrads():
    if STEP.token_pending:
        stages = [p_["stage"] for p_ in STEP.token_pending.values()]
        raise RuntimeError(f"a parked encoder-input backward chain was never completed (stages {stages}): gradients of this "
                           "step are invalid -- set MOBGT_NO_TOKEN_BWD_CHAIN=1 and report")
    items, hop, psum, tok, wide = STEP.wgrad_items, STEP.wgrad_hop, STEP.wgrad_psum, STEP.wgrad_stock_tok, STEP.wgrad_hop_wide
    STEP.wgrad_items, STEP.wgrad_hop, STEP.wgrad_psum, STEP.wgrad_stock_tok, STEP.wgrad_hop_wide = [], None, [], None, None
    for o in range(0, len(psum), 48):
        part = psum[o:o + 48]
        n = len(part)
        _lib.call("mobgt_partial_sum_multi", n, (ctypes.c_void_p * n)(*[p_[0].data_ptr() for p_ in part]),
                  (ctypes.c_void_p * n)(*[p_[1].data_ptr() for p_ in part]),
                  (ctypes.c_int * n)(*[p_[0].shape[0] for p_ in part]),
                  (ctypes.c_int64 * n)(*[p_[1].numel() for p_ in part]), _stream())
    if tok is not None and wide is not None:
        dtab, ew, dw_, d_ew, d_dw, D, E, rt = wide
        _lib.call("mobgt_stock_tail_bwd", *tok[0], _p(dtab), _p(ew), _p(dw_), _p(d_ew), _p(d_dw), D, E, 8, rt, _stream())
    elif tok is not None:
        _lib.call("mobgt_stock_tokens_bwd", *tok[0], _stream())
    elif wide is not None:
        _hop_table_bwd(wide)
    vp, i64, ci, cf = ctypes.c_void_p, ctypes.c_int64, ctypes.c_int, ctypes.c_float
    if hop is not None and not items:
        _hop_table_bwd(hop)
        hop = None
    for o in range(0, len(items), 32):
        part = items[o:o + 32]
        n = len(part)
        if hop is not None:
            dtab, ew, dw_, d_ew, d_dw, D, E, rt = hop
            hop_args = [1, _p(dtab), _p(ew), _p(dw_), _p(d_ew), _p(d_dw), D, E, rt]
            hop = None
        else:
            hop_args = [0, None, None, None, None, None, 0, 0, 0]
        ptr = lambda t: t.data_ptr() if t is not None else None
        mv = []
        for it in part:
            mv += list(it[4])
        _lib.call("mobgt_linear_wgrad_multi_hop",
            n, (vp * n)(*[ptr(it[0]) for it in part]), (i64 * n)(*[it[0].stride(0) for it in part]),
            (vp * n)(*[ptr(it[1]) for it in part]), (i64 * n)(*[it[1].stride(0) for it in part]),
            (vp * n)(*[ptr(it[2]) for it in part]), (vp * n)(*[ptr(it[3]) for it in part]), (cf * (3 * n))(*mv),
            (vp * n)(*[ptr(it[5]) for it in part]), (i64 * n)(*[it[5].stride(0) for it in part]),
            (vp * n)(*[ptr(it[6]) for it in part]), (ci * n)(*[int(it[7]) for it in part]),
            (i64 * n)(*[it[0].shape[0] for it in part]), (ci * n)(*[it[0].shape[1] for it in part]),
            (ci * n)(*[it[1].shape[1] for it in part]), (ci * n)(*[1 if it[0].dtype == torch.float32 else 0 for it in part]),
            *hop_args, _stream())


def linear_wgrad_masked(g, x, g_mask=None, x_mask=None, mask_vals=(1.0, 1.0, 1.0), db=None, db_of_x=False, dw=None, g_out=None,
                        leaf=False):
    _require_cuda(g, x)
    R, M = g.shape
    N = x.shape[1]
    assert g.dtype == torch.float32 and x.dtype == torch.float32 and g.stride(1) == 1 and x.stride(1) == 1
    for m, t in ((g_mask, g), (x_mask, x)):
        assert m is None or (m.dtype == torch.float32 and m.shape == t.shape and m.stride() == t.stride())
    if dw is None:
        dw = zeros_f32((M, N), g.device)
    assert g_out is None or (g_mask is not None and g_out.shape == g.shape and g_out.stride() == g.stride())
    if leaf and STEP.wgrad_on and g_out is None and M % 2 == 0 and N % 2 == 0:
        return _wgrad_defer(g, x, g_mask, x_mask, mask_vals, dw, db, db_of_x)
    _lib.call("mobgt_linear_wgrad_masked", _p(g), g.stride(0), _p(x), x.stride(0), _p(g_mask), _p(x_mask), float(mask_vals[0]),
              float(mask_vals[1]), float(mask_vals[2]), _p(g_out), _p(dw), N, _p(db), int(db_of_x),
              R, M, N, _stream())
    return dw


def small_gemm_ok(a, b):
    return (a.is_cuda and a.dtype == torch.float32 and b.dtype == torch.float32 and a.dim() == 2 and b.dim() == 2
            and a.stride(1) == 1 and b.stride(1) == 1)


GEMM_BIAS, GEMM_GELU, GEMM_GELU_BWD, GEMM_ADD = (_lib.CONSTANTS["MOBGT_GEMM_" + n] for n in ("BIAS", "GELU", "GELU_BWD", "ADD"))


def layer_gemm_ok(a, b, b_is_kn=False):
    if a.dtype != torch.bfloat16 or b.dtype != torch.bfloat16 or a.dim() != 2 or b.dim() != 2:
        return False
    M, K = a.shape
    N = b.shape[1] if b_is_kn else b.shape[0]
    if (b.shape[0] if b_is_kn else b.shape[1]) != K:
        return False
    return (K % 32 == 0 and N % 8 == 0 and a.stride(1) == 1 and b.stride(1) == 1 and a.stride(0) % 8 == 0
            and b.stride(0) % (2 if b_is_kn else 8) == 0 and a.data_ptr() % 16 == 0 and b.data_ptr() % 16 == 0
            and M <= 4096)


def layer_gemm(a, b, bias=None, b_is_kn=False, epilogue=GEMM_BIAS, aux_in=None):
    _require_cuda(a, b)
    M, K = a.shape
    N = b.shape[1] if b_is_kn else b.shape[0]
    dev = a.device
    aux_out = None
    if epilogue == GEMM_ADD:
        assert aux_in.dtype == torch.float32 and aux_in.shape == (M, N) and aux_in.is_contiguous()
        c = aux_in
    else:
        c = torch.empty(M, N, dtype=torch.bfloat16, device=dev)
        if epilogue == GEMM_GELU:
            aux_out = torch.empty(M, N, dtype=torch.bfloat16, device=dev)
        elif epilogue == GEMM_GELU_BWD:
            assert aux_in.dtype == torch.bfloat16 and aux_in.shape == (M, N) and aux_in.is_contiguous()
    if bias is not None:
        assert bias.dtype == torch.bfloat16 and bias.numel() == N and bias.is_contiguous()
    _lib.call("mobgt_layer_gemm", _p(a), a.stride(0), _p(b), b.stride(0), int(b_is_kn), _p(bias), _p(c), N, epilogue,
              _p(aux_in), _p(aux_out), M, N, K, _stream())
    return (c, aux_out) if epilogue == GEMM_GELU else c


_NAN_TRACE = {"flags": None, "names": [], "on": False}


def nan_trace_enable(device, slots=256):
    _NAN_TRACE.update(flags=torch.zeros(slots, dtype=torch.float32, device=device), names=[], on=True)


def trace_nan(name, t, grad=True):
    if not _NAN_TRACE["on"] or t is None:
        return t
    names, flags = _NAN_TRACE["names"], _NAN_TRACE["flags"]
    if name not in names:
        names.append(name)
        if grad:
            names.append("d/" + name)
    i = names.index(name)
    flags[i:i + 1].copy_(torch.isnan(t.detach()).any().float().reshape(1))
    if grad and t.requires_grad:
        j = names.index("d/" + name)
        def _hook(g, j=j):
            flags[j:j + 1].copy_(torch.isnan(g).any().float().reshape(1))
            return None
        t.register_hook(_hook)
    return t


def nan_trace_report():
    f = _NAN_TRACE["flags"].cpu().tolist()
    return [(n, bool(f[i])) for i, n in enumerate(_NAN_TRACE["names"])]


def linear_wgrad(g, x, with_bias=False, db=None, out_bias=None, leaf=False, dw=None):
    _require_cuda(g)
    R, M = g.shape
    N = x.shape[1]
    assert g.dtype == x.dtype and g.dtype in (torch.bfloat16, torch.float32) and g.stride(1) == 1 and x.stride(1) == 1
    if dw is None:
        dw = zeros_f32((M, N), g.device)
    if out_bias is not None:
        assert db is None and not with_bias and out_bias.dtype == torch.float32 and out_bias.numel() == N
        _lib.call("mobgt_linear_wgrad_bias", _p(g), g.stride(0), _p(x), x.stride(0), _p(out_bias.contiguous()), _p(dw), N, R, M, N,
                  _DT[g.dtype], _stream())
        return dw, None
    if db is None and with_bias:
        db = zeros_f32((M,), g.device)
    if leaf and STEP.wgrad_on and M % 2 == 0 and N % 2 == 0:
        return _wgrad_defer(g, x, None, None, (1.0, 1.0, 1.0), dw, db, False), (db[:] if db is not None else None)
    _lib.call("mobgt_linear_wgrad", _p(g), g.stride(0), _p(x), x.stride(0), _p(dw), N, _p(db), R, M, N, _DT[g.dtype],
              _stream())
    return dw, db


def colsum(g):
    _require_cuda(g)
    g = g.contiguous()
    R, C = g.shape
    out = zeros_f32((C,), g.device)
    _lib.call("mobgt_colsum", _p(g), _p(out), R, C, _DT[g.dtype], _stream())
    return out
```

mobgt_amd/step_state.py:

```python
import contextlib
from collections import namedtuple

PARKED, CARRIED, SWITCH = "parked", "carried", "switch"
Field = namedtuple("Field", "name scope new doc")
_none = type(None)

FIELDS = (
    Field("zero_arena", SWITCH, _none, "TrainStep._prologue sets the step's ZeroArena; ops.zeros_f32 carves from it"),
    Field("grad_sinks", CARRIED, dict, "TrainStep (ops.set_grad_sinks): parameter address -> (weak parameter, gradient view); ops.grad_sink reads"),
    Field("sink_census", SWITCH, lambda: {"on": False, "cur": {}, "max": {}}, "train.used_parameters' dry run counts ops.grad_sink requests per forward"),
    Field("bias_bwd_job", PARKED, _none, "_BuildBiasFn.forward parks; the category GCN's backward launch, the side stream or its own backward takes"),
    Field("front_on", SWITCH, bool, "the model's forward (ops.front_deferral) around the hop table and the node indices"),
    Field("front_hop", PARKED, _none, "_HopTableFn.forward parks; the category GCN's / stock front's forward launch or ops.flush_front takes"),
    Field("front_ni", PARKED, _none, "ops.node_index parks; the same launches take"),
    Field("token_fwd_on", SWITCH, bool, "model_fqandtoyo.node_features (ops.token_fwd_deferral)"),
    Field("token_fwd", PARKED, dict, "'gather' / 'f2' / 'f4': _GatherMultiFn / _LinearSplitKFn.forward record; _AssembleTokensFn launches them as one"),
    Field("token_fwd_fused_calls", CARRIED, int, "how often mobgt_token_fwd_chain took the three records (a counter for tests)"),
    Field("token_chain", CARRIED, _none, "ops.register_token_chain: the encoder-input chain of the forward that just ran; its backward reads it"),
    Field("token_pending", PARKED, dict, "_AssembleTokensFn.backward parks under a gradient's address; FuseEmbeddings-4 / -2's backward re-park / launch"),
    Field("front_sgemm", PARKED, dict, "'job': ops.front_small_gemm parks, the bias assembly's launch takes; 'done': its result until ops.small_gemm asks"),
    Field("wgrad_on", SWITCH, bool, "ops.recording_wgrads around the trainer's backward"),
    Field("wgrad_items", PARKED, list, "leaf weight gradients (ops.linear_wgrad*, fused layers) for ops.flush_deferred_wgrads' grouped launch"),
    Field("wgrad_hop", PARKED, _none, "_HopTableFn.backward parks; rides in the flush's first grouped launch"),
    Field("wgrad_hop_wide", PARKED, _none, "_HopTableFn.backward past 256 edge ids; shares the flush's stock tail launch"),
    Field("wgrad_stock_tok", PARKED, _none, "_StockTokensFn.backward parks; the flush's stock tail launch takes"),
    Field("wgrad_psum", PARKED, list, "ops.defer_partial_sum: split-K partial sums for the flush's one reduction launch"),
    Field("layer_tails", PARKED, dict, "(graph task, device, address of dx1) -> a fused layer's tail; the chain launch of the layer below takes"),
    Field("tail_check_task", PARKED, _none, "graph task whose end-of-backward check (fused_layer._pending_check) is queued"),
    Field("weight_pack", PARKED, list, "model.pack_layer_weights(defer=True) parks; the category GCN's / stock front's forward launch takes"),
    Field("gcn_prelaunched", PARKED, dict, "modelGNN.prelaunch_small_gcn: id(module) -> (key, result); that module's forward adopts it"),
)


class StepState:
    def __init__(self):
        for f in FIELDS:
            setattr(self, f.name, f.new())

    def leftovers(self):
        held = {f.name: getattr(self, f.name) for f in FIELDS if f.scope == PARKED}
        return {k: sorted(map(str, v)) if isinstance(v, dict) else len(v) if isinstance(v, list) else type(v).__name__
                for k, v in held.items() if v is not None and v != [] and v != {}}

    def drop_stale_tails(self, task_id):
        if self.tail_check_task != task_id:
            self.tail_check_task = None
        for k in [k for k in self.layer_tails if k[0] != task_id]:
            del self.layer_tails[k]

    def drop_parked(self, task_id=-1):
        self.drop_stale_tails(task_id)
        for f in FIELDS:
            if f.scope == PARKED and f.name not in ("layer_tails", "tail_check_task"):
                setattr(self, f.name, f.new())

    @contextlib.contextmanager
    def keeping_carried(self):
        saved = {f.name: getattr(self, f.name) for f in FIELDS if f.scope == CARRIED}
        try:
            yield
        finally:
            for k, v in saved.items():
                setattr(self, k, v)


STEP = StepState()
```

Baseline: 26930.

## Fuse embedding-gather scatter backward into the token backward chain kernel

Result: no change. 27190, median of 6 (+1.0%).

```diff
diff --git a/__graft_entry__.py b/__graft_entry__.py
--- a/__graft_entry__.py
+++ b/__graft_entry__.py
@@ -18,6 +18,9 @@
     from mobgt_amd import _universe
     _universe.LIBRARY.build()
     _universe.LIBRARY.lib()
+    from mobgt_amd import _tokbwd
+    _tokbwd.LIBRARY.build()
+    _tokbwd.LIBRARY.lib()
     subprocess.check_call(["make", "-s", "-C", os.path.join(ROOT, "oracle")])
     import mobgt_amd
 
diff --git a/include/mobgt_tokbwd.h b/include/mobgt_tokbwd.h
--- /dev/null
+++ b/include/mobgt_tokbwd.h
@@ -0,0 +1,30 @@
+#ifndef MOBGT_TOKBWD_H
+#define MOBGT_TOKBWD_H
+#include <stdint.h>
+
+#ifdef __cplusplus
+extern "C" {
+#endif
+
+#define MOBGT_TOKBWD_EBADDIM (-1)
+#define MOBGT_TOKBWD_EALIGN (-2)
+#define MOBGT_TOKBWD_EDTYPE (-3)
+
+#define MOBGT_TOKBWD_I64 0
+#define MOBGT_TOKBWD_I32 1
+
+#define MOBGT_TOKBWD_ABI_VERSION 1
+int mobgt_tokbwd_abi_version(void);
+
+int mobgt_token_bwd_chain_scatter(const float* dout, const float* real, const float* y4, const float* y2, int64_t ld_y2,
+                                  const float* w4, const float* w2, float* d_nf, float* d_add, float* dx4, int64_t ld_dx4,
+                                  float* d_pt, float* d_token, int G, int N, int C, int W2, float slope4, float slope2,
+                                  float p_pos, float p_in, uint64_t seed, const uint64_t* seed_dev, uint32_t salt_nf,
+                                  uint32_t salt_tok, uint32_t salt_in, int n_sc, float* const* sc_tables,
+                                  const void* const* sc_idx, const int64_t* sc_skip, const int* sc_width, const int* sc_coff,
+                                  const int* sc_src, int idx_dtype, int extra_job, void* stream);
+
+#ifdef __cplusplus
+}
+#endif
+#endif
diff --git a/mobgt_amd/_tokbwd.py b/mobgt_amd/_tokbwd.py
--- /dev/null
+++ b/mobgt_amd/_tokbwd.py
@@ -0,0 +1,13 @@
+from ._native import Library, NativeError
+
+
+class MobgtTokBwdError(NativeError):
+    pass
+
+
+LIBRARY = Library("mobgt_tokbwd.h", "csrc_tokbwd", "libmobgt_tokbwd.so", "MOBGT_TOKBWD_", error=MobgtTokBwdError,
+                  missing="the encoder input's backward with its hosted scatter runs on the device only.",
+                  errors={"EBADDIM": "unsupported dimension or job", "EALIGN": "alignment violation", "EDTYPE": "unknown dtype code"})
+lib, launch = LIBRARY.lib, LIBRARY.launch
+SIGNATURES, CONSTANTS, ABI_VERSION = LIBRARY.SIGNATURES, LIBRARY.CONSTANTS, LIBRARY.ABI_VERSION
+EBADDIM, EALIGN, EDTYPE, I64, I32 = LIBRARY.constants("EBADDIM", "EALIGN", "EDTYPE", "I64", "I32")
diff --git a/mobgt_amd/csrc/tokbwd.hip b/mobgt_amd/csrc/tokbwd.hip
--- a/mobgt_amd/csrc/tokbwd.hip
+++ b/mobgt_amd/csrc/tokbwd.hip
@@ -1,177 +1,4 @@
-#include "common.h"
-#include "mobgt_hip.h"
-
-namespace {
-
-typedef __attribute__((ext_vector_type(4))) float f32x4;
-
-constexpr int TNW = 12, TNT = TNW * 64, TBM = 16;
-
-struct TokBwdParams {
-    const float* dout;
-    const float* real;
-    const float* y4;
-    const float* y2; int64_t ld2;
-    const float *w4, *w2;
-    float *d_nf, *d_add;
-    float* dx4; int64_t ldx4;
-    float* d_pt;
-    float* d_token;
-    int G, N;
-    float slope4, slope2;
-    uint32_t thr_pos, thr_in;
-    float keep_pos, keep_in;
-    uint64_t seed;
-    const uint64_t* seed_dev;
-    uint32_t salt_nf, salt_tok, salt_in;
-    int n_node_blocks;
-};
-
-__device__ __forceinline__ float leaky_grad(float y, float slope) { return y > 0.f ? 1.f : slope; }
-
-#ifdef TB_STAMP
-__device__ int* g_tb_dbg = nullptr;
-#define TSTAMP_DECL int st_[8] = {}
-#define TSTAMP(i) st_[i] = (int)wall_clock64()
-#define TSTAMP_DUMP() do { if (g_tb_dbg && threadIdx.x == 0) for (int q_ = 0; q_ < 8; ++q_) g_tb_dbg[blockIdx.x * 8 + q_] = st_[q_]; } while (0)
-#else
-#define TSTAMP_DECL
-#define TSTAMP(i)
-#define TSTAMP_DUMP()
-#endif
-
-template <int N> constexpr int gemm_ks() { return TNW / ((N + 63) / 64); }
-template <int K, int N, int LDA, int LDO>
-__device__ __forceinline__ void gemm_kn(const float* __restrict__ A, const float* __restrict__ W, float* __restrict__ out) {
-    constexpr int NB = (N + 63) / 64, KS = TNW / NB, NT16 = K / 16, TMAX = (NT16 + KS - 1) / KS;
-    static_assert(K % 16 == 0 && N % 32 == 0 && KS >= 1, "shape");
-    const int lane = threadIdx.x & 63, wave = threadIdx.x >> 6;
-    const int j = lane & 15, q = lane >> 4;
-    if (wave >= NB * KS) return;
-    const int blk = wave / KS, ks = wave % KS;
-    const int t_lo = ks * NT16 / KS, t_hi = (ks + 1) * NT16 / KS;
-    const int n0 = 64 * blk;
-    const bool col_ok = n0 + 4 * j < N;
-    const int cl = col_ok ? n0 + 4 * j : 0;
-    f32x4 acc[4];
-#pragma unroll
-    for (int n = 0; n < 4; ++n) acc[n] = f32x4{0.f, 0.f, 0.f, 0.f};
-    f32x4 bw[TMAX][4];
-#pragma unroll
-    for (int tt = 0; tt < TMAX; ++tt) {
-        const int t = min(t_lo + tt, t_hi - 1);
-#pragma unroll
-        for (int i = 0; i < 4; ++i) bw[tt][i] = *reinterpret_cast<const f32x4*>(W + (int64_t)(16 * t + 4 * q + i) * N + cl);
-    }
-#pragma unroll
-    for (int tt = 0; tt < TMAX; ++tt) {
-        if (t_lo + tt < t_hi) {
-            const f32x4 a = *reinterpret_cast<const f32x4*>(A + j * LDA + 16 * (t_lo + tt) + 4 * q);
-#pragma unroll
-            for (int i = 0; i < 4; ++i)
-#pragma unroll
-                for (int n = 0; n < 4; ++n) acc[n] = __builtin_amdgcn_mfma_f32_16x16x4f32(a[i], bw[tt][i][n], acc[n], 0, 0, 0);
-        }
-    }
-    if (col_ok) {
-#pragma unroll
-        for (int n = 0; n < 4; ++n)
-#pragma unroll
-            for (int v = 0; v < 4; ++v) out[(ks * TBM + 4 * q + v) * LDO + n0 + 4 * j + n] = acc[n][v];
-    }
-}
-
-template <int C, int W2>
-__global__ __launch_bounds__(TNT) void token_bwd_chain_kernel(const TokBwdParams p) {
-    constexpr int LDA = C + 4, LD2 = W2 + 4;
-    __shared__ __attribute__((aligned(16))) float a4[TBM * LDA];
-    constexpr int KS4 = gemm_ks<C>(), KS2 = gemm_ks<W2>();
-    __shared__ __attribute__((aligned(16))) float t4[(KS4 > KS2 ? KS4 : KS2) * TBM * LDA];
-    const int lane = threadIdx.x & 63, wave = threadIdx.x >> 6;
-    const int T = p.N + 1;
-    const uint64_t seed = (p.thr_pos || p.thr_in) ? p.seed + (p.seed_dev ? *p.seed_dev : 0ull) : 0ull;
-    if ((int)blockIdx.x >= p.n_node_blocks) {
-        const int g = ((int)blockIdx.x - p.n_node_blocks) * TNW + wave;
-        if (g >= p.G) return;
-        const int64_t row = (int64_t)g * T;
-        const uint32_t h1 = p.thr_pos ? dropout_row_hash(seed, (uint32_t)g ^ p.salt_tok) : 0u;
-        const uint32_t h2 = p.thr_in ? dropout_row_hash(seed, (uint32_t)row ^ p.salt_in) : 0u;
-        for (int c = lane; c < C; c += 64) {
-            float scale = 1.f;
-            if (p.thr_pos) scale = dropout_bits16(seed, h1, (uint32_t)c) >= p.thr_pos ? p.keep_pos : 0.f;
-            if (p.thr_in) scale *= dropout_bits16(seed, h2, (uint32_t)c) >= p.thr_in ? p.keep_in : 0.f;
-            const float d = p.dout[row * C + c] * scale;
-            if (d != 0.f) atomicAdd(&p.d_token[c], d);
-        }
-        return;
-    }
-    const int64_t R = (int64_t)p.G * p.N;
-    const int64_t j0 = (int64_t)blockIdx.x * TBM;
-    TSTAMP_DECL;
-    TSTAMP(0);
-    constexpr int EPT = TBM * C / TNT;
-    static_assert(TBM * C % TNT == 0, "flat split");
-    float dv[EPT], yv[EPT], rl[EPT];
-#pragma unroll
-    for (int k = 0; k < EPT; ++k) {
-        const int e = threadIdx.x + k * TNT, r = e / C, c = e % C;
-        const int64_t jc = min(j0 + r, R - 1);
-        const int g = (int)(jc / p.N), n = (int)(jc - (int64_t)g * p.N);
-        dv[k] = p.dout[((int64_t)g * T + n + 1) * C + c];
-        yv[k] = p.y4[jc * C + c];
-        rl[k] = p.real[jc];
-    }
-#pragma unroll
-    for (int k = 0; k < EPT; ++k) {
-        const int e = threadIdx.x + k * TNT, r = e / C, c = e % C;
-        const int64_t jn = j0 + r;
-        const bool on = jn < R;
-        const int64_t jc = on ? jn : R - 1;
-        const int g = (int)(jc / p.N), n = (int)(jc - (int64_t)g * p.N);
-        const int64_t row = (int64_t)g * T + n + 1;
-        float scale = 1.f;
-        if (p.thr_pos) scale = dropout_bits16(seed, dropout_row_hash(seed, (uint32_t)jc ^ p.salt_nf), (uint32_t)c) >= p.thr_pos ? p.keep_pos : 0.f;
-        if (p.thr_in) scale *= dropout_bits16(seed, dropout_row_hash(seed, (uint32_t)row ^ p.salt_in), (uint32_t)c) >= p.thr_in ? p.keep_in : 0.f;
-        const float d = on ? dv[k] * scale : 0.f;
-        const float dnf = d * rl[k];
-        a4[r * LDA + c] = dnf * leaky_grad(yv[k], p.slope4);
-        if (on) {
-            p.d_add[jn * C + c] = d;
-            p.d_nf[jn * C + c] = dnf;
-        }
-    }
-    __syncthreads();
-    TSTAMP(1);
-    gemm_kn<C, C, LDA, LDA>(a4, p.w4, t4);
-    __syncthreads();
-    TSTAMP(2);
-    for (int e = threadIdx.x; e < TBM * C; e += TNT) {
-        const int r = e / C, c = e % C;
-        const int64_t jn = j0 + r;
-        float v = 0.f;
-#pragma unroll
-        for (int ks = 0; ks < KS4; ++ks) v += t4[(ks * TBM + r) * LDA + c];
-        if (jn < R) p.dx4[jn * p.ldx4 + c] = v;
-        if (c < W2) a4[r * LD2 + c] = jn < R ? v * leaky_grad(p.y2[jn * p.ld2 + c], p.slope2) : 0.f;
-    }
-    __syncthreads();
-    TSTAMP(3);
-    gemm_kn<W2, W2, LD2, LD2>(a4, p.w2, t4);
-    __syncthreads();
-    TSTAMP(4);
-    for (int e = threadIdx.x; e < TBM * W2; e += TNT) {
-        const int r = e / W2, c = e % W2;
-        const int64_t jn = j0 + r;
-        float v = 0.f;
-#pragma unroll
-        for (int ks = 0; ks < KS2; ++ks) v += t4[(ks * TBM + r) * LD2 + c];
-        if (jn < R) p.d_pt[jn * W2 + c] = v;
-    }
-    TSTAMP(5);
-    TSTAMP_DUMP();
-}
-
-}
+#include "tokbwd_body.h"
 
 #ifdef TB_STAMP
 extern "C" int mobgt_tokbwd_debug_buffer(int* buf) { return (int)hipMemcpyToSymbol(HIP_SYMBOL(g_tb_dbg), &buf, sizeof(buf)); }
@@ -182,19 +9,6 @@
                                      float* d_pt, float* d_token, int G, int N, int C, int W2, float slope4, float slope2,
                                      float p_pos, float p_in, uint64_t seed, const uint64_t* seed_dev, uint32_t salt_nf,
                                      uint32_t salt_tok, uint32_t salt_in, void* stream) {
-    if (G <= 0 || N <= 0) return MOBGT_EBADDIM;
-    if (!(C == 192 && W2 == 160)) return MOBGT_EBADDIM;
-    if (((uintptr_t)w4 | (uintptr_t)w2) & 15) return MOBGT_EALIGN;
-    TokBwdParams p = {};
-    p.dout = dout; p.real = real; p.y4 = y4; p.y2 = y2; p.ld2 = ld_y2; p.w4 = w4; p.w2 = w2; p.d_nf = d_nf; p.d_add = d_add;
-    p.dx4 = dx4; p.ldx4 = ld_dx4; p.d_pt = d_pt; p.d_token = d_token; p.G = G; p.N = N; p.slope4 = slope4; p.slope2 = slope2;
-    p.thr_pos = p_pos > 0.f ? dropout_threshold(p_pos) : 0u;
-    p.thr_in = p_in > 0.f ? dropout_threshold(p_in) : 0u;
-    p.keep_pos = p.thr_pos ? 1.f / (1.f - (float)p.thr_pos / 65536.f) : 1.f;
-    p.keep_in = p.thr_in ? 1.f / (1.f - (float)p.thr_in / 65536.f) : 1.f;
-    p.seed = seed; p.seed_dev = seed_dev; p.salt_nf = salt_nf; p.salt_tok = salt_tok; p.salt_in = salt_in;
-    p.n_node_blocks = (int)(((int64_t)G * N + TBM - 1) / TBM);
-    const dim3 grid(p.n_node_blocks + (G + TNW - 1) / TNW), block(TNT);
-    hipLaunchKernelGGL((token_bwd_chain_kernel<192, 160>), grid, block, 0, (hipStream_t)stream, p);
-    return (int)hipGetLastError();
+    return token_bwd_launch<false>(dout, real, y4, y2, ld_y2, w4, w2, d_nf, d_add, dx4, ld_dx4, d_pt, d_token, G, N, C, W2, slope4, slope2,
+                            p_pos, p_in, seed, seed_dev, salt_nf, salt_tok, salt_in, nullptr, stream);
 }
diff --git a/mobgt_amd/csrc/tokbwd_body.h b/mobgt_amd/csrc/tokbwd_body.h
--- /dev/null
+++ b/mobgt_amd/csrc/tokbwd_body.h
@@ -0,0 +1,270 @@
+#pragma once
+#include "common.h"
+#include "mobgt_hip.h"
+
+namespace {
+
+typedef __attribute__((ext_vector_type(4))) float f32x4;
+
+constexpr int TNW = 12, TNT = TNW * 64, TBM = 16;
+constexpr int SC_MAXJ = 8;
+enum { SRC_PT = 0, SRC_X4 = 1, SRC_ADD = 2 };
+
+struct TokScatter {
+    float* d_table[SC_MAXJ];
+    const void* idx[SC_MAXJ];
+    int64_t skip[SC_MAXJ];
+    int width[SC_MAXJ], coff[SC_MAXJ], src[SC_MAXJ];
+    int n, i64;
+    float* extra_row0;
+};
+
+struct TokBwdParams {
+    const float* dout;
+    const float* real;
+    const float* y4;
+    const float* y2; int64_t ld2;
+    const float *w4, *w2;
+    float *d_nf, *d_add;
+    float* dx4; int64_t ldx4;
+    float* d_pt;
+    float* d_token;
+    int G, N;
+    float slope4, slope2;
+    uint32_t thr_pos, thr_in;
+    float keep_pos, keep_in;
+    uint64_t seed;
+    const uint64_t* seed_dev;
+    uint32_t salt_nf, salt_tok, salt_in;
+    int n_node_blocks;
+    TokScatter sc;
+};
+
+__device__ __forceinline__ float leaky_grad(float y, float slope) { return y > 0.f ? 1.f : slope; }
+
+#ifdef TB_STAMP
+__device__ int* g_tb_dbg = nullptr;
+#define TSTAMP_DECL int st_[8] = {}
+#define TSTAMP(i) st_[i] = (int)wall_clock64()
+#define TSTAMP_DUMP() do { if (g_tb_dbg && threadIdx.x == 0) for (int q_ = 0; q_ < 8; ++q_) g_tb_dbg[blockIdx.x * 8 + q_] = st_[q_]; } while (0)
+#else
+#define TSTAMP_DECL
+#define TSTAMP(i)
+#define TSTAMP_DUMP()
+#endif
+
+template <int N> constexpr int gemm_ks() { return TNW / ((N + 63) / 64); }
+template <int K, int N, int LDA, int LDO>
+__device__ __forceinline__ void gemm_kn(const float* __restrict__ A, const float* __restrict__ W, float* __restrict__ out) {
+    constexpr int NB = (N + 63) / 64, KS = TNW / NB, NT16 = K / 16, TMAX = (NT16 + KS - 1) / KS;
+    static_assert(K % 16 == 0 && N % 32 == 0 && KS >= 1, "shape");
+    const int lane = threadIdx.x & 63, wave = threadIdx.x >> 6;
+    const int j = lane & 15, q = lane >> 4;
+    if (wave >= NB * KS) return;
+    const int blk = wave / KS, ks = wave % KS;
+    const int t_lo = ks * NT16 / KS, t_hi = (ks + 1) * NT16 / KS;
+    const int n0 = 64 * blk;
+    const bool col_ok = n0 + 4 * j < N;
+    const int cl = col_ok ? n0 + 4 * j : 0;
+    f32x4 acc[4];
+#pragma unroll
+    for (int n = 0; n < 4; ++n) acc[n] = f32x4{0.f, 0.f, 0.f, 0.f};
+    f32x4 bw[TMAX][4];
+#pragma unroll
+    for (int tt = 0; tt < TMAX; ++tt) {
+        const int t = min(t_lo + tt, t_hi - 1);
+#pragma unroll
+        for (int i = 0; i < 4; ++i) bw[tt][i] = *reinterpret_cast<const f32x4*>(W + (int64_t)(16 * t + 4 * q + i) * N + cl);
+    }
+#pragma unroll
+    for (int tt = 0; tt < TMAX; ++tt) {
+        if (t_lo + tt < t_hi) {
+            const f32x4 a = *reinterpret_cast<const f32x4*>(A + j * LDA + 16 * (t_lo + tt) + 4 * q);
+#pragma unroll
+            for (int i = 0; i < 4; ++i)
+#pragma unroll
+                for (int n = 0; n < 4; ++n) acc[n] = __builtin_amdgcn_mfma_f32_16x16x4f32(a[i], bw[tt][i][n], acc[n], 0, 0, 0);
+        }
+    }
+    if (col_ok) {
+#pragma unroll
+        for (int n = 0; n < 4; ++n)
+#pragma unroll
+            for (int v = 0; v < 4; ++v) out[(ks * TBM + 4 * q + v) * LDO + n0 + 4 * j + n] = acc[n][v];
+    }
+}
+
+template <int C, int W2, bool SC>
+__global__ __launch_bounds__(TNT) void token_bwd_chain_kernel(const TokBwdParams p) {
+    constexpr int LDA = C + 4, LD2 = W2 + 4;
+    __shared__ __attribute__((aligned(16))) float a4[TBM * LDA];
+    constexpr int KS4 = gemm_ks<C>(), KS2 = gemm_ks<W2>();
+    __shared__ __attribute__((aligned(16))) float t4[(KS4 > KS2 ? KS4 : KS2) * TBM * LDA];
+    const int lane = threadIdx.x & 63, wave = threadIdx.x >> 6;
+    const int T = p.N + 1;
+    const uint64_t seed = (p.thr_pos || p.thr_in) ? p.seed + (p.seed_dev ? *p.seed_dev : 0ull) : 0ull;
+    if ((int)blockIdx.x >= p.n_node_blocks) {
+        const int g = ((int)blockIdx.x - p.n_node_blocks) * TNW + wave;
+        if (g >= p.G) return;
+        const int64_t row = (int64_t)g * T;
+        const uint32_t h1 = p.thr_pos ? dropout_row_hash(seed, (uint32_t)g ^ p.salt_tok) : 0u;
+        const uint32_t h2 = p.thr_in ? dropout_row_hash(seed, (uint32_t)row ^ p.salt_in) : 0u;
+        for (int c = lane; c < C; c += 64) {
+            float scale = 1.f;
+            if (p.thr_pos) scale = dropout_bits16(seed, h1, (uint32_t)c) >= p.thr_pos ? p.keep_pos : 0.f;
+            if (p.thr_in) scale *= dropout_bits16(seed, h2, (uint32_t)c) >= p.thr_in ? p.keep_in : 0.f;
+            const float d = p.dout[row * C + c] * scale;
+            if (d != 0.f) atomicAdd(&p.d_token[c], d);
+            if (SC && d != 0.f && p.sc.extra_row0) atomicAdd(&p.sc.extra_row0[c], d);
+        }
+        return;
+    }
+    const int64_t R = (int64_t)p.G * p.N;
+    const int64_t j0 = (int64_t)blockIdx.x * TBM;
+    __shared__ int64_t sc_rows[SC ? SC_MAXJ : 1][TBM];
+    if (SC) {
+#pragma unroll
+        for (int t = 0; t < SC_MAXJ; ++t) {
+            if (t >= p.sc.n) break;
+            const int r = (int)threadIdx.x - t * TBM;
+            if (r < 0 || r >= TBM) continue;
+            int64_t row = -1;
+            if (j0 + r < R && p.sc.d_table[t]) {
+                row = p.sc.i64 ? reinterpret_cast<const int64_t*>(p.sc.idx[t])[j0 + r] : (int64_t)reinterpret_cast<const int32_t*>(p.sc.idx[t])[j0 + r];
+                if (row == p.sc.skip[t]) row = -1;
+            }
+            sc_rows[t][r] = row;
+        }
+    }
+    TSTAMP_DECL;
+    TSTAMP(0);
+    constexpr int EPT = TBM * C / TNT;
+    static_assert(TBM * C % TNT == 0, "flat split");
+    float dv[EPT], yv[EPT], rl[EPT], dk[SC ? EPT : 1];
+#pragma unroll
+    for (int k = 0; k < EPT; ++k) {
+        const int e = threadIdx.x + k * TNT, r = e / C, c = e % C;
+        const int64_t jc = min(j0 + r, R - 1);
+        const int g = (int)(jc / p.N), n = (int)(jc - (int64_t)g * p.N);
+        dv[k] = p.dout[((int64_t)g * T + n + 1) * C + c];
+        yv[k] = p.y4[jc * C + c];
+        rl[k] = p.real[jc];
+    }
+#pragma unroll
+    for (int k = 0; k < EPT; ++k) {
+        const int e = threadIdx.x + k * TNT, r = e / C, c = e % C;
+        const int64_t jn = j0 + r;
+        const bool on = jn < R;
+        const int64_t jc = on ? jn : R - 1;
+        const int g = (int)(jc / p.N), n = (int)(jc - (int64_t)g * p.N);
+        const int64_t row = (int64_t)g * T + n + 1;
+        float scale = 1.f;
+        if (p.thr_pos) scale = dropout_bits16(seed, dropout_row_hash(seed, (uint32_t)jc ^ p.salt_nf), (uint32_t)c) >= p.thr_pos ? p.keep_pos : 0.f;
+        if (p.thr_in) scale *= dropout_bits16(seed, dropout_row_hash(seed, (uint32_t)row ^ p.salt_in), (uint32_t)c) >= p.thr_in ? p.keep_in : 0.f;
+        const float d = on ? dv[k] * scale : 0.f;
+        const float dnf = d * rl[k];
+        a4[r * LDA + c] = dnf * leaky_grad(yv[k], p.slope4);
+        if (on) {
+            p.d_add[jn * C + c] = d;
+            p.d_nf[jn * C + c] = dnf;
+        }
+        if (SC) dk[k] = d;
+    }
+    __syncthreads();
+    TSTAMP(1);
+    gemm_kn<C, C, LDA, LDA>(a4, p.w4, t4);
+    __syncthreads();
+    TSTAMP(2);
+    for (int e = threadIdx.x; e < TBM * C; e += TNT) {
+        const int r = e / C, c = e % C;
+        const int64_t jn = j0 + r;
+        float v = 0.f;
+#pragma unroll
+        for (int ks = 0; ks < KS4; ++ks) v += t4[(ks * TBM + r) * LDA + c];
+        if (jn < R) p.dx4[jn * p.ldx4 + c] = v;
+        if (SC && c >= W2) a4[TBM * LD2 + r * (C - W2) + c - W2] = v;
+        if (c < W2) a4[r * LD2 + c] = jn < R ? v * leaky_grad(p.y2[jn * p.ld2 + c], p.slope2) : 0.f;
+    }
+    __syncthreads();
+    TSTAMP(3);
+    gemm_kn<W2, W2, LD2, LD2>(a4, p.w2, t4);
+    __syncthreads();
+    TSTAMP(4);
+    for (int e = threadIdx.x; e < TBM * W2; e += TNT) {
+        const int r = e / W2, c = e % W2;
+        const int64_t jn = j0 + r;
+        float v = 0.f;
+#pragma unroll
+        for (int ks = 0; ks < KS2; ++ks) v += t4[(ks * TBM + r) * LD2 + c];
+        if (jn < R) p.d_pt[jn * W2 + c] = v;
+        if (SC) t4[r * LD2 + c] = v;
+    }
+    if (SC) {
+        static_assert(TBM * LD2 + TBM * (C - W2) <= TBM * LDA && KS2 >= 2 && KS4 >= 2, "tiles");
+        float* dt = t4 + TBM * LDA;
+        __syncthreads();
+#pragma unroll
+        for (int k = 0; k < EPT; ++k) {
+            const int e = threadIdx.x + k * TNT;
+            dt[(e / C) * LDA + e % C] = dk[k];
+        }
+        __syncthreads();
+        int base = 0;
+#pragma unroll
+        for (int t = 0; t < SC_MAXJ; ++t) {
+            if (t >= p.sc.n) break;
+            const int W = p.sc.width[t], coff = p.sc.coff[t], src = p.sc.src[t];
+            int cc = (int)threadIdx.x - base % TNT;
+            if (cc < 0) cc += TNT;
+            base += W;
+            if (!p.sc.d_table[t]) continue;
+            const float* tile = src == SRC_PT ? t4 + coff : (src == SRC_X4 ? a4 + TBM * LD2 + coff - W2 : dt + coff);
+            const int ld = src == SRC_PT ? LD2 : (src == SRC_X4 ? C - W2 : LDA);
+            for (; cc < W; cc += TNT) {
+                float* dst = p.sc.d_table[t] + cc;
+                int64_t cur = -1;
+                float acc = 0.f;
+#pragma unroll
+                for (int r = 0; r < TBM; ++r) {
+                    const int64_t row = sc_rows[t][r];
+                    if (row != cur) {
+                        if (cur >= 0) atomicAdd(dst + cur * W, acc);
+                        cur = row;
+                        acc = 0.f;
+                    }
+                    if (row >= 0) acc += tile[r * ld + cc];
+                }
+                if (cur >= 0) atomicAdd(dst + cur * W, acc);
+            }
+        }
+    }
+    TSTAMP(5);
+    TSTAMP_DUMP();
+}
+
+}
+
+
+template <bool SC>
+static int token_bwd_launch(const float* dout, const float* real, const float* y4, const float* y2, int64_t ld_y2, const float* w4,
+                            const float* w2, float* d_nf, float* d_add, float* dx4, int64_t ld_dx4, float* d_pt, float* d_token,
+                            int G, int N, int C, int W2, float slope4, float slope2, float p_pos, float p_in, uint64_t seed,
+                            const uint64_t* seed_dev, uint32_t salt_nf, uint32_t salt_tok, uint32_t salt_in, const TokScatter* sc,
+                            void* stream) {
+    if (G <= 0 || N <= 0) return MOBGT_EBADDIM;
+    if (!(C == 192 && W2 == 160)) return MOBGT_EBADDIM;
+    if (((uintptr_t)w4 | (uintptr_t)w2) & 15) return MOBGT_EALIGN;
+    TokBwdParams p = {};
+    p.dout = dout; p.real = real; p.y4 = y4; p.y2 = y2; p.ld2 = ld_y2; p.w4 = w4; p.w2 = w2; p.d_nf = d_nf; p.d_add = d_add;
+    p.dx4 = dx4; p.ldx4 = ld_dx4; p.d_pt = d_pt; p.d_token = d_token; p.G = G; p.N = N; p.slope4 = slope4; p.slope2 = slope2;
+    p.thr_pos = p_pos > 0.f ? dropout_threshold(p_pos) : 0u;
+    p.thr_in = p_in > 0.f ? dropout_threshold(p_in) : 0u;
+    p.keep_pos = p.thr_pos ? 1.f / (1.f - (float)p.thr_pos / 65536.f) : 1.f;
+    p.keep_in = p.thr_in ? 1.f / (1.f - (float)p.thr_in / 65536.f) : 1.f;
+    p.seed = seed; p.seed_dev = seed_dev; p.salt_nf = salt_nf; p.salt_tok = salt_tok; p.salt_in = salt_in;
+    p.n_node_blocks = (int)(((int64_t)G * N + TBM - 1) / TBM);
+    const dim3 grid(p.n_node_blocks + (G + TNW - 1) / TNW), block(TNT);
+    if (SC) p.sc = *sc;
+    hipLaunchKernelGGL((token_bwd_chain_kernel<192, 160, SC>), grid, block, 0, (hipStream_t)stream, p);
+    return (int)hipGetLastError();
+}
diff --git a/mobgt_amd/csrc_tokbwd/scatter.hip b/mobgt_amd/csrc_tokbwd/scatter.hip
--- /dev/null
+++ b/mobgt_amd/csrc_tokbwd/scatter.hip
@@ -0,0 +1,35 @@
+#include "../csrc/tokbwd_body.h"
+#include "mobgt_tokbwd.h"
+
+static_assert(MOBGT_TOKBWD_EBADDIM == MOBGT_EBADDIM && MOBGT_TOKBWD_EALIGN == MOBGT_EALIGN && MOBGT_TOKBWD_EDTYPE == MOBGT_EDTYPE &&
+              MOBGT_TOKBWD_I64 == MOBGT_I64 && MOBGT_TOKBWD_I32 == MOBGT_I32, "the shared launcher returns libmobgt_hip's codes");
+
+extern "C" int mobgt_tokbwd_abi_version(void) { return MOBGT_TOKBWD_ABI_VERSION; }
+
+extern "C" int mobgt_token_bwd_chain_scatter(const float* dout, const float* real, const float* y4, const float* y2, int64_t ld_y2,
+                                             const float* w4, const float* w2, float* d_nf, float* d_add, float* dx4,
+                                             int64_t ld_dx4, float* d_pt, float* d_token, int G, int N, int C, int W2, float slope4,
+                                             float slope2, float p_pos, float p_in, uint64_t seed, const uint64_t* seed_dev,
+                                             uint32_t salt_nf, uint32_t salt_tok, uint32_t salt_in, int n_sc,
+                                             float* const* sc_tables, const void* const* sc_idx, const int64_t* sc_skip,
+                                             const int* sc_width, const int* sc_coff, const int* sc_src, int idx_dtype,
+                                             int extra_job, void* stream) {
+    if (n_sc < 0 || n_sc > SC_MAXJ || extra_job >= n_sc) return MOBGT_EBADDIM;
+    if (idx_dtype != MOBGT_TOKBWD_I64 && idx_dtype != MOBGT_TOKBWD_I32) return MOBGT_EDTYPE;
+    TokScatter sc = {};
+    sc.n = n_sc; sc.i64 = idx_dtype == MOBGT_TOKBWD_I64;
+    for (int t = 0; t < n_sc; ++t) {
+        if (sc_src[t] == SRC_X4 && sc_coff[t] < W2) return MOBGT_EBADDIM;
+        const int wsrc = sc_src[t] == SRC_PT ? W2 : ((sc_src[t] == SRC_X4 || sc_src[t] == SRC_ADD) ? C : -1);
+        if (wsrc < 0 || sc_width[t] <= 0 || sc_coff[t] < 0 || sc_coff[t] + sc_width[t] > wsrc || !sc_idx[t]) return MOBGT_EBADDIM;
+        sc.d_table[t] = sc_tables ? sc_tables[t] : nullptr;
+        sc.idx[t] = sc_idx[t]; sc.skip[t] = sc_skip ? sc_skip[t] : -1;
+        sc.width[t] = sc_width[t]; sc.coff[t] = sc_coff[t]; sc.src[t] = sc_src[t];
+    }
+    if (extra_job >= 0) {
+        if (sc.width[extra_job] != C) return MOBGT_EBADDIM;
+        sc.extra_row0 = sc.d_table[extra_job];
+    }
+    return token_bwd_launch<true>(dout, real, y4, y2, ld_y2, w4, w2, d_nf, d_add, dx4, ld_dx4, d_pt, d_token, G, N, C, W2, slope4, slope2,
+                            p_pos, p_in, seed, seed_dev, salt_nf, salt_tok, salt_in, &sc, stream);
+}
diff --git a/mobgt_amd/forms.py b/mobgt_amd/forms.py
--- a/mobgt_amd/forms.py
+++ b/mobgt_amd/forms.py
@@ -20,6 +20,8 @@
     Form("skinny_all", "MOBGT_SKINNY_ALL", False, "all three classifier products on csrc/skinny.hip (off: dW / db only)"),
     Form("token_fwd_chain", "MOBGT_NO_TOKEN_FWD_CHAIN", True, "the encoder input's forward as one launch (off: four)"),
     Form("token_bwd_chain", "MOBGT_NO_TOKEN_BWD_CHAIN", True, "the encoder input's backward as one launch, csrc/tokbwd.hip (off: three)"),
+    Form("token_scatter", "MOBGT_NO_TOKEN_SCATTER", True, "inside a train step: the gathered rows' scatter-add, in the encoder input's "
+         "backward launch (off: the gather node's own backward launch)"),
     Form("pack_passenger", "MOBGT_NO_PACK_PASSENGER", True, "the layers' weight pack, in the next front launch"),
     Form("front_passengers", "MOBGT_NO_FRONT_PASSENGERS", True, "hop table forward and node-feature indices, in the category GCN's forward"),
     Form("bias_bwd_passenger", "MOBGT_NO_BIAS_BWD_PASSENGER", True, "short batches: the bias tables' backward, in the category GCN's backward"),
diff --git a/mobgt_amd/ops.py b/mobgt_amd/ops.py
--- a/mobgt_amd/ops.py
+++ b/mobgt_amd/ops.py
@@ -4,7 +4,7 @@
 
 import torch
 
-from . import _lib, forms
+from . import _lib, _tokbwd, forms
 from ._lib import F32, BF16, I64, I32, I16, U8, check
 from .step_state import STEP
 
@@ -1261,6 +1261,14 @@
         ctx.ptrs = [t.data_ptr() for t in tables]
         ctx.shapes = [t.shape for t in tables]
         ctx.sinks = [grad_sink(t) for t in tables]
+        ctx.rec = None
+        req = [bool(r_) for r_ in ctx.needs_input_grad[3:3 + n]]
+        if (STEP.zero_arena is not None and STEP.grad_sinks and any(req) and sum(req) <= 8 and forms.on("token_scatter")
+                and forms.on("token_bwd_chain") and len(outs) == 3 and all(i_.dtype == idx[0].dtype for i_ in idx)
+                and idx[0].dtype in (torch.int64, torch.int32) and all(sp[0] in (0, 1, 2) for sp in spec)):
+            ctx.rec = dict(idx=idx, spec=spec, sinks=ctx.sinks, shapes=ctx.shapes, ptrs=ctx.ptrs, R=R, req=req,
+                           outs=[o.data_ptr() for o in outs], grads=None, bufs=None)
+        STEP.token_scatter = ctx.rec
         return tuple(outs)
 
     @staticmethod
@@ -1268,6 +1276,17 @@
         n, spec = ctx.n, ctx.spec
         dev = ctx.idx[0].device
         R = ctx.idx[0].numel()
+        rec = ctx.rec
+        if rec is not None:
+            if STEP.token_scatter is rec:
+                STEP.token_scatter = None
+            if rec["grads"] is not None:
+                if any(g is None or g.data_ptr() != b for g, b in zip(douts, rec["bufs"])):
+                    raise RuntimeError("mobgt: the gathered rows' gradients were scattered by the encoder input's backward launch, "
+                                       "but other gradients arrived at the gather (do the gathered rows have a second consumer?); "
+                                       "set MOBGT_NO_TOKEN_SCATTER=1")
+                grads = [rec["grads"][t][:] if (t in rec["grads"] and ctx.needs_input_grad[3 + t]) else None for t in range(n)]
+                return (None, None, None, *grads, *([None] * n))
         gbuf = []
         for g in douts:
             if g is not None and (g.stride(1) != 1 or g.stride(0) % 4 or g.data_ptr() % 16 or g.dtype != torch.float32):
@@ -1513,7 +1532,33 @@
                                 w2=w2.detach(), slope2=float(slope2))
 
 
-def _token_park_linear(g, w, y):
+def _token_scatter_jobs(pend, x, d_pt, dx4):
+    rec, ent = STEP.token_scatter, pend["ent"]
+    if (rec is None or rec["grads"] is not None or not forms.on("token_scatter")
+            or rec["outs"] != [x.data_ptr(), ent["x4"].data_ptr(), pend["add_ptr"]] or rec["R"] != ent["nf"].shape[0]):
+        return None
+    spec, jobs = rec["spec"], [t for t, r_ in enumerate(rec["req"]) if r_]
+    extra_job = -1
+    for k, t in enumerate(jobs):
+        row0 = _ROW0_PENDING.get(rec["ptrs"][t])
+        if row0 is not None:
+            if row0.data_ptr() != pend["d_tok"].data_ptr() or rec["shapes"][t][1] != ent["nf"].shape[1]:
+                return None
+            extra_job = k
+    for t in jobs:
+        _ROW0_PENDING.pop(rec["ptrs"][t], None)
+    dev = x.device
+    grads = {t: (rec["sinks"][t][:] if rec["sinks"][t] is not None else zeros_f32(tuple(rec["shapes"][t]), dev)) for t in jobs}
+    rec["grads"], rec["bufs"] = grads, [d_pt.data_ptr(), dx4.data_ptr(), pend["d_add"].data_ptr()]
+    m = len(jobs)
+    ci, i64, vp = ctypes.c_int, ctypes.c_int64, ctypes.c_void_p
+    return (m, (vp * m)(*[grads[t].data_ptr() for t in jobs]), (vp * m)(*[rec["idx"][t].data_ptr() for t in jobs]),
+            (i64 * m)(*[spec[t][3] for t in jobs]), (ci * m)(*[rec["shapes"][t][1] for t in jobs]),
+            (ci * m)(*[spec[t][1] for t in jobs]), (ci * m)(*[spec[t][0] for t in jobs]),
+            _tokbwd.I64 if rec["idx"][0].dtype == torch.int64 else _tokbwd.I32, extra_job)
+
+
+def _token_park_linear(g, w, y, x=None):
     pend = STEP.token_pending.get(g.data_ptr())
     if pend is None:
         return None
@@ -1530,10 +1575,15 @@
         W2 = ent["w2"].shape[0]
         d_pt = torch.empty(G * N, W2, dtype=torch.float32, device=g.device)
         dx4 = pend["dx4"]
-        _lib.call("mobgt_token_bwd_chain", _p(pend["dout"]), _p(pend["real"]), _p(ent["nf"]), _p(ent["x4"]), ent["x4"].stride(0),
-                  _p(ent["w4"]), _p(ent["w2"]), _p(pend["d_nf"]), _p(pend["d_add"]), _p(dx4), dx4.stride(0),
-                  _p(d_pt), _p(pend["d_tok"]), G, N, C, W2, ent["slope4"], ent["slope2"], p_pos, p_in, seed,
-                  _p(seed_dev), salts[0], salts[1], salts[2], _stream())
+        sc = _token_scatter_jobs(pend, x, d_pt, dx4) if x is not None else None
+        args = (_p(pend["dout"]), _p(pend["real"]), _p(ent["nf"]), _p(ent["x4"]), ent["x4"].stride(0),
+                _p(ent["w4"]), _p(ent["w2"]), _p(pend["d_nf"]), _p(pend["d_add"]), _p(dx4), dx4.stride(0),
+                _p(d_pt), _p(pend["d_tok"]), G, N, C, W2, ent["slope4"], ent["slope2"], p_pos, p_in, seed,
+                _p(seed_dev), salts[0], salts[1], salts[2])
+        if sc is None:
+            _lib.call("mobgt_token_bwd_chain", *args, _stream())
+        else:
+            _tokbwd.launch("mobgt_token_bwd_chain_scatter", *args, *sc, _stream())
         return d_pt
     return None
 
@@ -1587,14 +1637,14 @@
                     and max(w.shape) <= 512):
                 db = dst(k_b, (g.shape[1],))
                 dw = linear_wgrad_masked(g, x, g_mask=y, mask_vals=mv, db=db, leaf=True, dw=dst(k_w, tuple(w.shape)))
-                dx = _token_park_linear(g, w, y) if STEP.wgrad_on else None
+                dx = _token_park_linear(g, w, y, x) if STEP.wgrad_on else None
                 return (dx if dx is not None else small_gemm(g, w, a_mask=(y, *mv))), dw, (db[:] if STEP.wgrad_on else db), None, None, None
             if (STEP.wgrad_on and hip_wgrad and g.stride(1) == 1 and y.stride() == g.stride() and g.data_ptr() % 8 == 0
                     and y.data_ptr() % 8 == 0 and g.stride(0) % 2 == 0 and small_gemm_ok(g, w) and R <= _SMALL_ROWS
                     and max(w.shape) <= 512):
                 db = dst(k_b, (g.shape[1],))
                 dw = linear_wgrad_masked(g, x, g_mask=y, mask_vals=mv, db=db, leaf=True, dw=dst(k_w, tuple(w.shape)))
-                dx = _token_park_linear(g, w, y)
+                dx = _token_park_linear(g, w, y, x)
                 return (dx if dx is not None else small_gemm(g, w, a_mask=(y, *mv))), dw, db[:], None, None, None
             if (hip_wgrad and g.stride(1) == 1 and y.stride() == g.stride() and g.data_ptr() % 8 == 0 and y.data_ptr() % 8 == 0
                     and g.stride(0) % 2 == 0):
@@ -1897,6 +1947,7 @@
         ctx.nf_ptr = nf.data_ptr()
         G, N, C = nf.shape
         nf, add, real = nf.contiguous(), add.contiguous(), real.contiguous()
+        ctx.add_ptr = add.data_ptr()
         shapes = (token.shape, pe0.shape)
         token = token.reshape(-1).contiguous()
         pe0 = pe0.contiguous() if pe0.dim() == 2 and pe0.shape[0] > 1 else pe0.reshape(-1).contiguous()
@@ -1941,7 +1992,7 @@
         if (ent is not None and ent["nf_ptr"] == ctx.nf_ptr and STEP.wgrad_on and C == ent["nf"].shape[1]
                 and G * N == ent["nf"].shape[0] and forms.on("token_bwd_chain")):
             STEP.token_pending[d_nf.data_ptr()] = dict(stage=1, ent=ent, dout=dout, real=real, d_nf=d_nf, d_add=d_add, d_tok=d_tok,
-                                                       misc=(G, N, C, p_pos, p_in, seed, seed_dev, salts))
+                                                       add_ptr=ctx.add_ptr, misc=(G, N, C, p_pos, p_in, seed, seed_dev, salts))
         else:
             _lib.call("mobgt_assemble_tokens_bwd", _p(dout), _p(real), _p(d_nf), _p(d_add), _p(d_tok), G, N, C, p_pos, p_in, seed,
                       _p(seed_dev), salts[0], salts[1], salts[2], _stream())
diff --git a/mobgt_amd/step_state.py b/mobgt_amd/step_state.py
--- a/mobgt_amd/step_state.py
+++ b/mobgt_amd/step_state.py
@@ -18,6 +18,8 @@
     Field("token_fwd_fused_calls", CARRIED, int, "how often mobgt_token_fwd_chain took the three records (a counter for tests)"),
     Field("token_chain", CARRIED, _none, "ops.register_token_chain: the encoder-input chain of the forward that just ran; its backward reads it"),
     Field("token_pending", PARKED, dict, "_AssembleTokensFn.backward parks under a gradient's address; FuseEmbeddings-4 / -2's backward re-park / launch"),
+    Field("token_scatter", PARKED, _none, "_GatherMultiFn.forward parks its jobs inside a train step; ops._token_park_linear's launch scatters them "
+          "and leaves the tables' gradients in the record; _GatherMultiFn.backward takes it"),
     Field("front_sgemm", PARKED, dict, "'job': ops.front_small_gemm parks, the bias assembly's launch takes; 'done': its result until ops.small_gemm asks"),
     Field("wgrad_on", SWITCH, bool, "ops.recording_wgrads around the trainer's backward"),
     Field("wgrad_items", PARKED, list, "leaf weight gradients (ops.linear_wgrad*, fused layers) for ops.flush_deferred_wgrads' grouped launch"),
```
